# aquaskyline/SOAPdenovo-Trans

Hardware: AMD Instinct MI355X
Metric: pregraph k-mers hashed/sec (higher is better)
Workload: dtype u64

## Files before the change

soapdenovo-trans_amd/csrc/sdt_pipeline.hip:

```cpp
#include "sdt_ctx.hpp"
#include "sdt_tile.cuh"
#include "sdt_superkmer_kernels.cuh"
#include "sdt_count_plan.h"
#include "sdt_pipeline.hpp"

void sk_free(sdt_ctx *c)
{
	sdt_ctx::SkState &k = c->sk;
	void *dev[] = {k.p1.recs, k.p1.meta, k.p1.next, k.p2.recs, k.p2.meta, k.p2.next, k.cursors, k.blk, k.cnt1, k.off1, k.fill1, k.list1,
	               k.cnt2, k.off2, k.fill2, k.list2, k.kmers2, k.kpre2, k.items, k.citems, k.next_item};
	for (void *p : dev)
		if (p) (void)hipFree(p);
	void *host[] = {k.h_off1, k.h_off2, k.h_kpre2, k.h_items, k.h_citems};
	for (void *p : host)
		if (p) (void)hipHostFree(p);
	const uint64_t in_total = k.l2_in_total;
	const bool exchanged = k.exchanged;
	const uint32_t stream_flushes = k.stream_flushes;
	k = sdt_ctx::SkState();
	k.l2_in_total = in_total;
	k.exchanged = exchanged;
	k.stream_flushes = stream_flushes;
}

SkGeo sk_geo(int K, uint64_t max_read_len)
{
	SkGeo g;
	g.mtw = (int)(((uint64_t)SK_TILE_READS * max_read_len + 16 + 15) / 16) + TAIL_PAD + 1;
	g.tile_words = (int)((tile_smem_bytes(g.mtw) / sizeof(uint32_t) + 1) & ~(size_t)1);
	g.hv_words = (int)((SK_TILE_READS * max_read_len + 16 + 1) & ~(uint64_t)1);
	const uint64_t nk_max = (uint64_t)SK_TILE_READS * (max_read_len - K + 1);
	g.bits_words = (int)(nk_max / 64 + 2);
	g.hv2_words = K - sk_minimizer_len(K) + 1 > 49 ? g.hv_words : 0;
	g.smem = (size_t)g.tile_words * 4 + (size_t)SK_NB1 * 8 + (size_t)(g.hv_words + g.hv2_words) * 4 + (size_t)g.bits_words * 8 + (size_t)(g.bits_words + 2) * 4;
	return g;
}

template <int NW, bool TRACK> static size_t sk_count_smem()
{
	using G = SkCntGeo<NW, TRACK>;
	constexpr int SLOTS = G::SLOTS, BW = SkFmt<NW>::BW, TR = G::TILE;
	return (size_t)(NW + (TRACK ? 1 : 0)) * SLOTS * 8 + (size_t)TR * 8 + (size_t)SLOTS * 20 + (size_t)TR * 4 + G::REGION +
	       (size_t)(LDS_LEAD + TR * BW * 2 + TAIL_PAD) * 4;
}

bool sk_applicable(const sdt_ctx *c, uint64_t max_read_len)
{
	if (c->flags & SDT_FLAG_CONTIG_INDEX)
		return false;
	if (max_read_len < (uint64_t)c->K + 1 || max_read_len > (uint64_t)SK_MAX_READ_LEN)
		return false;
	return sk_geo(c->K, max_read_len).smem <= 160 * 1024;
}

int sk_reset_pool1(sdt_ctx *c)
{
	sdt_ctx::SkState &k = c->sk;
	HIPCHK(hipMemsetAsync(k.p1.next, 0, 4, c->stream));
	HIPCHK(hipMemsetAsync(k.cnt1, 0, SK_NB1 * 4, c->stream));
	hipLaunchKernelGGL(k_sk_init_cursors, dim3(256), dim3(256), 0, c->stream, k.cursors, k.wgs * (uint32_t)SK_NB1, (uint32_t)SK_CAP1, k.blk, k.wgs);
	HIPCHK(hipGetLastError());
	k.pending_kmers = 0;
	return SDT_OK;
}

int sk_alloc(sdt_ctx *c, uint64_t want_kmers, uint64_t per_read)
{
	sdt_ctx::SkState &k = c->sk;
	if (want_kmers > SK_BATCH_MAX_KMERS)
		want_kmers = SK_BATCH_MAX_KMERS;
	if (k.ready && (k.cap_kmers >= want_kmers || k.cap_is_max || k.pending_kmers))
		return SDT_OK;
	if (k.ready) {
		HIPCHK(hipStreamSynchronize(c->stream));
		sk_free(c);
	}
	const bool compact = sk_compact(c);
	const int rw = sk_rec_words(c->nw), rw2 = sk_rec2_stride(c->nw, compact);
	const int w = c->K - sk_minimizer_len(c->K) + 1;
	const bool strips = c->nw == 4 || per_read > (uint64_t)SK_SEQ_MAX_KMERS;
	const int cap_c = strips ? sk_pow2_floor(sk_max_run(c->K, c->nw, compact)) : sk_max_run(c->K, c->nw, compact);
	const double rate = 2.0 / (double)(w + 1) + 1.0 / (double)sk_max_run(c->K, c->nw);
	const double more = compact ? (2.0 / (double)(w + 1) + 1.0 / (double)cap_c) / rate : 1.0;
	double run = 1.0 / rate * ((c->nw == 4 || per_read > (uint64_t)SK_SEQ_MAX_KMERS) ? 0.8 : 1.0);
	if (run > (double)per_read) run = (double)per_read;
	uint64_t div = (uint64_t)run;
	if (div < 2) div = 2;
	div = (uint64_t)clamp_int(sdt_knob_int(sdt_tuning_env("SDT_SK_POOL_DIV"), (int)div), 1, 1 << 20);
	const int mem_pct = sdt_knob_int(sdt_tuning_env("SDT_SK_POOL_MEM_PCT"), 70);
	size_t free_b = 0, total_b = 0;
	HIPCHK(sdti::mem_info(&free_b, &total_b));
	uint64_t cap = want_kmers < (1ULL << 24) ? (1ULL << 24) : want_kmers;
	k.cap_is_max = cap >= SK_BATCH_MAX_KMERS;
	const uint32_t wgs = (uint32_t)c->cu_count * 6;
	for (;; cap /= 2) {
		const uint64_t recs = (uint64_t)((double)(cap / div) * more);
		const uint64_t chunks1 = sdt_knob_int(sdt_test_env("SDT_SK_POOL_CHUNKS1"), 0) > 0 ? (uint64_t)sdt_knob_int(sdt_test_env("SDT_SK_POOL_CHUNKS1"), 0) : recs / SK_CAP1 + (uint64_t)wgs * SK_NB1 + 1024;
		const uint64_t items = chunks1 / SK_ITEM_CHUNKS + SK_NB1 + 1;
		const uint64_t chunks2 = chunks1 * (SK_CAP1 / SK_CAP2) + items * (SK_NB2 + SK_BLK2) + 1024;
		const uint64_t bytes = chunks1 * SK_CAP1 * rw * 8 + chunks2 * SK_CAP2 * rw2 * 8 + (chunks1 + chunks2) * 8;
		const uint64_t all = c->comm.nranks > 1 ? bytes + chunks1 * SK_CAP1 * rw * 8 * 9 / 2 : bytes;
		if (chunks2 >= (1ULL << SK_LIST2_FILL_SHIFT) - 1 || all > free_b / 100 * (uint64_t)mem_pct) {
			k.cap_is_max = true;
			if (cap <= (1ULL << 24))
				return fail(SDT_ENOMEM, "super-k-mer pools: %llu MiB needed for the smallest batch, %zu MiB free",
				            (unsigned long long)(bytes >> 20), free_b >> 20);
			continue;
		}
		k.p1.chunks = (uint32_t)chunks1;
		k.p2.chunks = (uint32_t)chunks2;
		k.items_cap = (uint32_t)items;
		break;
	}
	k.wgs = wgs;
	const double t_alloc0 = comm_now();
	HIPCHK(hipMalloc((void **)&k.p1.recs, (size_t)k.p1.chunks * SK_CAP1 * rw * 8));
	HIPCHK(hipMalloc((void **)&k.p1.meta, (size_t)k.p1.chunks * 4));
	HIPCHK(hipMalloc((void **)&k.p1.next, 64));
	HIPCHK(hipMalloc((void **)&k.p2.recs, (size_t)k.p2.chunks * SK_CAP2 * rw2 * 8));
	HIPCHK(hipMalloc((void **)&k.p2.meta, (size_t)k.p2.chunks * 4));
	HIPCHK(hipMalloc((void **)&k.p2.next, 64));
	HIPCHK(hipMalloc((void **)&k.cursors, (size_t)wgs * SK_NB1 * 8));
	HIPCHK(hipMalloc((void **)&k.blk, (size_t)wgs * 8));
	HIPCHK(hipMalloc((void **)&k.cnt1, SK_NB1 * 4));
	HIPCHK(hipMalloc((void **)&k.off1, (SK_NB1 + 1) * 4));
	HIPCHK(hipMalloc((void **)&k.fill1, SK_NB1 * 4));
	HIPCHK(hipMalloc((void **)&k.list1, (size_t)k.p1.chunks * 4));
	HIPCHK(hipMalloc((void **)&k.cnt2, SK_NBF * 4));
	HIPCHK(hipMalloc((void **)&k.off2, (SK_NBF + 1) * 4));
	HIPCHK(hipMalloc((void **)&k.fill2, SK_NBF * 4));
	HIPCHK(hipMalloc((void **)&k.list2, (size_t)k.p2.chunks * 4));
	HIPCHK(hipMalloc((void **)&k.kmers2, SK_NBF * 8));
	HIPCHK(hipMalloc((void **)&k.kpre2, (SK_NBF + 1) * 8));
	HIPCHK(hipMalloc((void **)&k.items, (size_t)k.items_cap * sizeof(SkItem)));
	HIPCHK(hipHostMalloc((void **)&k.h_off1, (SK_NB1 + 1) * 4, hipHostMallocDefault));
	HIPCHK(hipHostMalloc((void **)&k.h_off2, (SK_NBF + 1) * 4, hipHostMallocDefault));
	HIPCHK(hipHostMalloc((void **)&k.h_kpre2, (SK_NBF + 1) * 8, hipHostMallocDefault));
	HIPCHK(hipHostMalloc((void **)&k.h_items, (size_t)k.items_cap * sizeof(SkItem), hipHostMallocDefault));
	k.citems_cap = (uint32_t)SK_NBF + k.p2.chunks / SK_COUNT_ITEM_CHUNKS + 1;
	HIPCHK(hipMalloc((void **)&k.citems, (size_t)k.citems_cap * sizeof(uint4)));
	HIPCHK(hipHostMalloc((void **)&k.h_citems, (size_t)k.citems_cap * sizeof(uint4), hipHostMallocDefault));
	HIPCHK(hipMalloc((void **)&k.next_item, SK_MAX_COUNT_LAUNCHES * sizeof(uint32_t)));
	k.cap_kmers = cap;
	k.ready = true;
	if (sdt_env("SDT_TIMING"))
		fprintf(stderr, "[libsdt_gpu] super-k-mer pools for %llu k-mers per batch: %.1f GiB in %.0f ms\n", (unsigned long long)cap,
		        ((double)k.p1.chunks * SK_CAP1 * rw + (double)k.p2.chunks * SK_CAP2 * rw2) * 8 / (1 << 30), (comm_now() - t_alloc0) * 1e3);
	return sk_reset_pool1(c);
}

template <int NW, bool TRACK, bool COMPACT> static int sk_launch_count_t(sdt_ctx *c, uint32_t i0, uint32_t i1, uint32_t launch)
{
	sdt_ctx::SkState &k = c->sk;
	const size_t smem = sk_count_smem<NW, TRACK>();
	const unsigned per_cu = (unsigned)((160 * 1024) / (smem + 256));
	unsigned grid = (unsigned)c->cu_count * (per_cu < 1 ? 1 : (per_cu > 2 ? 2 : per_cu));
	if (grid > i1 - i0) grid = i1 - i0;
	HIPCHK(hipFuncSetAttribute((const void *)k_sk_count<NW, TRACK, COMPACT>, hipFuncAttributeMaxDynamicSharedMemorySize, (int)smem));
	hipLaunchKernelGGL((k_sk_count<NW, TRACK, COMPACT>), dim3(grid), dim3(SkCntGeo<NW, TRACK>::TPB), smem, c->stream, k.p2, k.list2, (const uint4 *)k.citems, i0, i1,
	                   k.next_item + launch, c->K, flat_of<NW>(c), c->d_stats);
	HIPCHK(hipGetLastError());
	return SDT_OK;
}

template <int NW> static int sk_launch_count(sdt_ctx *c, uint32_t i0, uint32_t i1, uint32_t launch)
{
	if (c->d_first)
		return sk_launch_count_t<NW, true, false>(c, i0, i1, launch);
	if constexpr (NW == 1)
		if (sk_compact(c))
			return sk_launch_count_t<1, false, true>(c, i0, i1, launch);
	return sk_launch_count_t<NW, false, false>(c, i0, i1, launch);
}


int sk_list1(sdt_ctx *c)
{
	sdt_ctx::SkState &k = c->sk;
	const int g = c->cu_count * 8;
	hipLaunchKernelGGL(k_sk_seal, dim3(256), dim3(256), 0, c->stream, k.cursors, k.wgs * (uint32_t)SK_NB1, k.blk, k.wgs, k.p1, (uint32_t)SK_CAP1);
	hipLaunchKernelGGL(k_sk_scan, dim3(1), dim3(1024), 0, c->stream, k.cnt1, k.off1, k.fill1, (int)SK_NB1, (const unsigned long long *)nullptr, (unsigned long long *)nullptr);
	hipLaunchKernelGGL(k_sk_chunk_place_few, dim3(g), dim3(256), 0, c->stream, k.p1, k.off1, k.fill1, k.list1, (int)SK_NB1);
	SK_CHK(hipGetLastError());
	SK_CHK(hipMemcpyAsync(k.h_off1, k.off1, (SK_NB1 + 1) * 4, hipMemcpyDeviceToHost, c->stream));
	{ const int rcw = c->comm.sync_watched(c->stream, "the chunk lists of a round"); if (rcw != SDT_OK) return rcw; }
	k.st_chunks1 = k.h_off1[SK_NB1];
	return SDT_OK;
}

int sk_split(sdt_ctx *c, const SkPool &src, const uint32_t *list, uint32_t nitems, hipEvent_t after_l2)
{
	sdt_ctx::SkState &k = c->sk;
	const int g = c->cu_count * 8;
	SK_CHK(hipMemsetAsync(k.p2.next, 0, 4, c->stream));
	SK_CHK(hipMemsetAsync(k.kmers2, 0, SK_NBF * 8, c->stream));
	SK_CHK(hipMemsetAsync(k.cnt2, 0, SK_NBF * 4, c->stream));
	if (nitems) {
		SK_CHK(hipMemcpyAsync(k.items, k.h_items, (size_t)nitems * sizeof(SkItem), hipMemcpyHostToDevice, c->stream));
#define SK_L2_LAUNCH(NW, COMPACT)                                                                                                   \
		do {                                                                                                                        \
			const size_t sm = SkL2Stage<NW, COMPACT>::SMEM;                                                                         \
			SK_CHK(hipFuncSetAttribute((const void *)k_sk_scatter_records_staged<NW, COMPACT>, hipFuncAttributeMaxDynamicSharedMemorySize, (int)sm)); \
			hipLaunchKernelGGL((k_sk_scatter_records_staged<NW, COMPACT>), dim3(nitems), dim3(SK_L2S_TPB), sm, c->stream, src, list, k.items, k.p2, k.cnt2, k.kmers2, c->d_stats); \
		} while (0)
		if (c->nw == 1 && sk_compact(c)) SK_L2_LAUNCH(1, true);
		else if (c->nw == 1) SK_L2_LAUNCH(1, false);
		else if (c->nw == 2) SK_L2_LAUNCH(2, false);
		else SK_L2_LAUNCH(4, false);
#undef SK_L2_LAUNCH
		SK_CHK(hipGetLastError());
	}
	if (after_l2)
		SK_CHK(hipEventRecord(after_l2, c->stream));
	hipLaunchKernelGGL(k_sk_scan, dim3(1), dim3(1024), 0, c->stream, k.cnt2, k.off2, k.fill2, (int)SK_NBF, (const unsigned long long *)k.kmers2, k.kpre2);
	hipLaunchKernelGGL(k_sk_chunk_place, dim3(g), dim3(256), 0, c->stream, k.p2, k.off2, k.fill2, k.list2);
	SK_CHK(hipGetLastError());
	SK_CHK(hipMemcpyAsync(k.h_kpre2, k.kpre2, (SK_NBF + 1) * 8, hipMemcpyDeviceToHost, c->stream));
	SK_CHK(hipMemcpyAsync(k.h_off2, k.off2, (SK_NBF + 1) * 4, hipMemcpyDeviceToHost, c->stream));
	return SDT_OK;
}

int sk_count_all(sdt_ctx *c)
{
	sdt_ctx::SkState &k = c->sk;
	SK_CHK(hipStreamSynchronize(c->stream));
	k.st_chunks2 = k.h_off2[SK_NBF];
	k.st_flushes++;
	k.stream_flushes++;
	k.l2_in_total += k.h_kpre2[SK_NBF];
	int rc = SDT_OK;
	uint32_t nci = 0;
	SK_CHK(hipMemsetAsync(k.next_item, 0, SK_MAX_COUNT_LAUNCHES * sizeof(uint32_t), c->stream));
	std::vector<uint32_t> first_item(SK_MAX_COUNT_LAUNCHES + 2);
	std::vector<uint64_t> launch_kmers(SK_MAX_COUNT_LAUNCHES + 2);
	uint32_t nlaunches = 0;
	
	if (!sk_plan_count_items(k.h_off2, (const uint64_t *)k.h_kpre2, (uint32_t)SK_NBF, c->kmers_known == 0 ? (1ULL << 26) : SK_COUNT_KMERS, SK_COUNT_KMERS,
	                         SK_MAX_COUNT_LAUNCHES, SK_COUNT_PACK_CHUNKS, SK_COUNT_ITEM_CHUNKS, (uint32_t *)k.h_citems, k.citems_cap,
	                         first_item.data(), launch_kmers.data(), (uint32_t)first_item.size(), &nci, &nlaunches))
		return fail(SDT_ESTATE, "count stage: work item table overflow");
	first_item.resize(nlaunches + 1);
	launch_kmers.resize(nlaunches);
	std::vector<uint32_t> sort_tmp;
	auto guess_of = [&](uint64_t kmers) -> uint64_t {
		uint64_t bound = kmers;
		if (c->kmers_known) {
			const double rate = (double)c->distinct_known / (double)c->kmers_known;
			const uint64_t guess = (uint64_t)((double)kmers * (2.0 * rate < 1.0 ? 2.0 * rate : 1.0)) + (1ULL << 22);
			if (guess < bound) bound = guess;
		}
		return bound;
	};
	const size_t nl = first_item.size() - 1;
	for (size_t l = 0; l < nl && rc == SDT_OK;) {
		const uint32_t i0 = first_item[l];
		if (i0 == first_item[l + 1]) {
			l++;
			continue;
		}
		if (c->kmers_known == 0 && l > 0) {
			rc = sync_stats(c);
			if (rc != SDT_OK) break;
		}
		uint64_t bound = guess_of(launch_kmers[l]), hard = launch_kmers[l];
		rc = ensure_room(c, bound);
		if (rc == SDT_OK && (double)(c->distinct_known + c->hard_since_sync + launch_kmers[l]) > 0.95 * (double)c->slots) {
			rc = sync_stats(c);
			if (rc == SDT_OK && (double)(c->distinct_known + launch_kmers[l]) > 0.95 * (double)c->slots)
				rc = grow_table(c, c->distinct_known + launch_kmers[l]);
		}
		size_t m = l;
		while (rc == SDT_OK && c->kmers_known && m + 1 < nl) {
			const uint64_t b2 = guess_of(launch_kmers[m + 1]);
			if ((double)(c->distinct_known + c->kmers_since_sync + bound + b2) > (double)c->slots * MAX_LOAD)
				break;
			if ((double)(c->distinct_known + c->hard_since_sync + hard + launch_kmers[m + 1]) > 0.95 * (double)c->slots)
				break;
			bound += b2;
			hard += launch_kmers[m + 1];
			m++;
		}
		const uint32_t i1 = first_item[m + 1];
		if (m > l)
			sk_plan_largest_first((uint32_t *)k.h_citems, i0, i1, sort_tmp);
		if (rc == SDT_OK)
			SK_CHK(hipMemcpyAsync(k.citems + i0, k.h_citems + i0, (size_t)(i1 - i0) * sizeof(uint4), hipMemcpyHostToDevice, c->stream));
		if (rc == SDT_OK)
			rc = c->nw == 1 ? sk_launch_count<1>(c, i0, i1, (uint32_t)l) : c->nw == 2 ? sk_launch_count<2>(c, i0, i1, (uint32_t)l) : sk_launch_count<4>(c, i0, i1, (uint32_t)l);
		if (rc == SDT_OK) {
			c->kmers_since_sync += bound;
			c->hard_since_sync += hard;
		}
		l = m + 1;
	}
	return rc;
}

int sk_add_items(sdt_ctx::SkState &k, uint32_t &nitems, uint32_t b, uint32_t lo, uint32_t hi)
{
	for (uint32_t c0 = lo; c0 < hi; c0 += SK_ITEM_CHUNKS) {
		if (nitems >= k.items_cap)
			return fail(SDT_EHIP, "super-k-mer pipeline: item table overflow");
		k.h_items[nitems++] = SkItem{b, c0, c0 + SK_ITEM_CHUNKS < hi ? c0 + SK_ITEM_CHUNKS : hi, 0};
	}
	return SDT_OK;
}

int sk_flush_sharded(sdt_ctx *c);

int sk_flush(sdt_ctx *c)
{
	sdt_ctx::SkState &k = c->sk;
	if (!k.ready || k.pending_kmers == 0 || k.flushing)
		return SDT_OK;
	if (c->comm.nranks > 1)
		return fail(SDT_ESTATE, "sharded context: the pipeline is drained by the collective calls (sdt_gpu_count_reads_sharded)");
	k.flushing = true;
	EventPair *ev = next_event(c), *ev2 = next_event(c);
	if (!ev || !ev2) { k.flushing = false; return fail(SDT_EHIP, "hipEventCreate failed"); }
	ev = ev2 - 1;
	ev->kmers = ev2->kmers = 0;
	ev->stage = SDT_STAGE_SK_SPLIT;
	ev2->stage = SDT_STAGE_SK_COUNT;
	int rc = hipEventRecord(ev->a, c->stream) == hipSuccess ? SDT_OK : fail(SDT_EHIP, "hipEventRecord failed");
	if (rc == SDT_OK) rc = sk_list1(c);
	uint32_t nitems = 0;
	for (uint32_t b = 0; b < (uint32_t)SK_NB1 && rc == SDT_OK; b++)
		rc = sk_add_items(k, nitems, b, k.h_off1[b], k.h_off1[b + 1]);
	if (rc == SDT_OK) rc = sk_split(c, k.p1, k.list1, nitems, nullptr);
	if (rc == SDT_OK) rc = sk_reset_pool1(c);
	if (rc == SDT_OK && (hipEventRecord(ev->b, c->stream) != hipSuccess || hipEventRecord(ev2->a, c->stream) != hipSuccess))
		rc = fail(SDT_EHIP, "hipEventRecord failed");
	if (rc == SDT_OK) {
		k.pending_kmers = 0;
		rc = sk_count_all(c);
	}
	if (hipEventRecord(ev2->b, c->stream) != hipSuccess && rc == SDT_OK)
		rc = fail(SDT_EHIP, "hipEventRecord failed");
	k.flushing = false;
	return rc;
}

template <int NW> static Table<NW> sk_tbl(const sdt_ctx *c, bool allow_direct)
{
	Table<NW> t = flat_of<NW>(c);
	if (!allow_direct)
		t.ent = nullptr;
	return t;
}

int sk_scatter_launch(sdt_ctx *c, const uint32_t *d_words, const uint64_t *d_offs, uint64_t nr, uint64_t max_read_len, uint64_t ob,
                             bool allow_direct)
{
	sdt_ctx::SkState &k = c->sk;
	const uint64_t per_read = max_read_len - c->K + 1;
	const SkGeo geo = sk_geo(c->K, max_read_len);
	const int m = sk_minimizer_len(c->K), ncap = sk_max_run(c->K, c->nw, sk_compact(c));
	const uint64_t ntiles = (nr + SK_TILE_READS - 1) / SK_TILE_READS;
	const unsigned grid = (unsigned)(ntiles < k.wgs ? ntiles : k.wgs);
	EventPair *ev = next_event(c);
	if (!ev)
		return fail(SDT_EHIP, "hipEventCreate failed");
	ev->kmers = nr * per_read;
	ev->stage = SDT_STAGE_SK_SCATTER;
	HIPCHK(hipEventRecord(ev->a, c->stream));
#define SK_SCATTER(NW)                                                                                                             \
	do {                                                                                                                       \
		HIPCHK(hipFuncSetAttribute((const void *)k_sk_scatter_reads<NW>, hipFuncAttributeMaxDynamicSharedMemorySize, (int)geo.smem)); \
		hipLaunchKernelGGL(k_sk_scatter_reads<NW>, dim3(grid), dim3(TPB), geo.smem, c->stream, d_words, d_offs, nr, c->K, m, sk_pow2_floor(ncap), \
		                   geo.mtw, geo.tile_words, geo.hv_words, geo.hv2_words, geo.bits_words, k.p1, k.cursors, k.blk, k.cnt1, sk_tbl<NW>(c, allow_direct), c->d_stats, ob, c->ord_stride); \
	} while (0)
	const int w = c->K - m + 1;
	static const bool no_seq = sdt_tuning_env("SDT_SK_STRIPS") != NULL;
	const bool seq1 = c->nw == 1 && (w & 1) && w >= 9 && w <= 21 && per_read <= (uint64_t)SK_SEQ_MAX_KMERS;
	const bool seq2 = c->nw == 2 && (w & 1) && w >= 23 && w <= 53 && per_read <= (uint64_t)SK_SEQ_MAX_KMERS;
	if ((seq1 || seq2) && !no_seq) {
		SkSeqLaunch a;
		a.words = d_words; a.offs = d_offs; a.nreads = nr; a.K = c->K; a.m = m; a.ncap = ncap;
		a.mtw = (int)(((uint64_t)SK_SEQ_TILE * max_read_len + 16 + 15) / 16) + TAIL_PAD + 1;
		a.pool = k.p1; a.cursors = k.cursors; a.blk = k.blk; a.cnt = k.cnt1; a.stats = c->d_stats;
		a.ord_base = ob; a.ord_stride = c->ord_stride; a.max_wgs = k.wgs; a.cu_count = c->cu_count; a.stream = c->stream;
		HIPCHK(seq1 ? sk_seq_launch_nw1(w, a, sk_tbl<1>(c, allow_direct)) : (w <= 33 ? sk_seq_launch_nw2_lo(w, a, sk_tbl<2>(c, allow_direct))
		            : (w <= 43 ? sk_seq_launch_nw2_mid(w, a, sk_tbl<2>(c, allow_direct)) : sk_seq_launch_nw2_hi(w, a, sk_tbl<2>(c, allow_direct)))));
	} else if (c->nw == 1) SK_SCATTER(1);
	else if (c->nw == 2) SK_SCATTER(2);
	else SK_SCATTER(4);
#undef SK_SCATTER
	HIPCHK(hipGetLastError());
	HIPCHK(hipEventRecord(ev->b, c->stream));
	k.pending_kmers += nr * per_read;
	return SDT_OK;
}

uint64_t sk_batch_limit(const sdt_ctx *c)
{
	const sdt_ctx::SkState &k = c->sk;
	if (c->expect_kmers && c->expect_kmers / 16 >= (1ULL << 27) && k.stream_flushes < 4) {
		const uint64_t lim = (c->expect_kmers / 16) << k.stream_flushes;
		if (lim < k.cap_kmers)
			return lim;
	}
	return k.cap_kmers;
}

int sk_scatter(sdt_ctx *c, const uint32_t *d_words, const uint64_t *d_offs, uint64_t nreads, uint64_t max_read_len)
{
	sdt_ctx::SkState &k = c->sk;
	const uint64_t per_read = max_read_len - c->K + 1;
	int rc = SDT_OK;
	if (k.ready && k.pending_kmers && !k.cap_is_max && k.cap_kmers < k.pending_kmers + nreads * per_read && k.cap_kmers < (1ULL << 31))
		rc = sk_flush(c);
	if (rc == SDT_OK) {
		uint64_t want = k.pending_kmers + nreads * per_read;
		if (!(c->flags & SDT_FLAG_PARTITION) && want < (1ULL << 31))
			want = 1ULL << 31;
		if (c->expect_kmers > want) {
			const uint64_t lim = 1ULL << clamp_int(sdt_knob_int(sdt_tuning_env("SDT_SK_HINT_BATCH_LOG2"), 32), 24, 34);
			const uint64_t hinted = c->expect_kmers < lim ? c->expect_kmers : lim;
			if (hinted > want) want = hinted;
		}
		rc = sk_alloc(c, want, per_read);
	}
	if (rc != SDT_OK)
		return rc;
	for (uint64_t r0 = 0; r0 < nreads;) {
		if (k.pending_kmers + per_read * SK_TILE_READS > sk_batch_limit(c)) {
			rc = sk_flush(c);
			if (rc == SDT_OK && !k.cap_is_max && k.cap_kmers < (1ULL << 31))
				rc = sk_alloc(c, k.cap_kmers * 2, per_read);
			if (rc != SDT_OK)
				return rc;
		}
		uint64_t nr = (sk_batch_limit(c) - k.pending_kmers) / per_read / SK_TILE_READS * SK_TILE_READS;
		if (nr > nreads - r0) nr = nreads - r0;
		rc = sk_scatter_launch(c, d_words, d_offs + r0, nr, max_read_len, c->ord_base + r0 * c->ord_stride);
		if (rc != SDT_OK)
			return rc;
		r0 += nr;
	}
	return SDT_OK;
}

extern "C" {
int sdt_sk_plan_count_items(const uint32_t *off2, const uint64_t *kpre2, uint32_t nbuckets, uint64_t first_limit, uint64_t limit,
                            uint32_t max_launches, uint32_t *items, uint32_t items_cap, uint32_t *first_item, uint64_t *launch_kmers,
                            uint32_t launches_cap, uint32_t *nitems, uint32_t *nlaunches)
{
	if (!off2 || !kpre2 || !items || !first_item || !launch_kmers || !nitems || !nlaunches)
		return fail(SDT_EINVAL, "NULL argument");
	if (max_launches < 1 || limit == 0 || first_limit == 0)
		return fail(SDT_EINVAL, "bad argument (at least one launch, limits of at least one k-mer)");
	if (!sk_plan_count_items(off2, kpre2, nbuckets, first_limit, limit, max_launches, SK_COUNT_PACK_CHUNKS, SK_COUNT_ITEM_CHUNKS, items, items_cap,
	                         first_item, launch_kmers, launches_cap, nitems, nlaunches))
		return fail(SDT_ENOMEM, "output arrays too small");
	return SDT_OK;
}

int sdt_kmer_bucket(const uint64_t *key_words_msw_first, int K)
{
	if (!key_words_msw_first || K < 13 || K > 127)
		return -1;
	const int nw = K <= 31 ? 1 : (K <= 63 ? 2 : 4), m = sk_minimizer_len(K);
	uint32_t best = 0xFFFFFFFFu;
	for (int p = 0; p + m <= K; p++) {
		uint32_t fw = 0;
		for (int i = 0; i < m; i++) {
			const int bit = 2 * (K - 1 - (p + i));
			const uint64_t w = key_words_msw_first[nw - 1 - bit / 64];
			fw = (fw << 2) | (uint32_t)((w >> (bit % 64)) & 3u);
		}
		const uint32_t hv = sk_mmer_hash(sk_canon_mmer(fw, m));
		if (hv < best) best = hv;
	}
	return (int)sk_l1_bucket(sk_bucket_hash(best));
}

int sdt_kmer_final_bucket(const uint64_t *key_words_msw_first, int K)
{
	if (!key_words_msw_first || K < 13 || K > 127)
		return -1;
	if (K <= 31) { Key<1> k{{key_words_msw_first[0]}}; return (int)key_final_bucket<1>(k, K); }
	if (K <= 63) { Key<2> k{{key_words_msw_first[0], key_words_msw_first[1]}}; return (int)key_final_bucket<2>(k, K); }
	Key<4> k{{key_words_msw_first[0], key_words_msw_first[1], key_words_msw_first[2], key_words_msw_first[3]}};
	return (int)key_final_bucket<4>(k, K);
}
#ifdef SDT_SK_L2_LOG
extern "C" int sdt_gpu_debug_l2_log(sdt_ctx *c, void *d_buf, uint64_t cap)
{
	unsigned long long *p = (unsigned long long *)d_buf, cp = cap;
	HIPCHK(hipSetDevice(c->device));
	HIPCHK(hipMemcpyToSymbol(HIP_SYMBOL(g_l2_log), &p, sizeof p));
	HIPCHK(hipMemcpyToSymbol(HIP_SYMBOL(g_l2_log_cap), &cp, sizeof cp));
	return SDT_OK;
}
#endif
}
```

soapdenovo-trans_amd/csrc/sdt_pipeline.hpp:

```cpp
#pragma once
#include "sdt_ctx.hpp"

static const uint64_t SK_BATCH_MAX_KMERS = 1ULL << clamp_int(sdt_knob_int(sdt_size_env("SDT_SK_BATCH_LOG2"), 35), 24, 36);
static const uint32_t SK_ITEM_CHUNKS = (uint32_t)clamp_int(sdt_knob_int(sdt_size_env("SDT_SK_ITEM_CHUNKS"), 4096), 16, 4096);
static const uint64_t SK_COUNT_KMERS = 1ULL << clamp_int(sdt_knob_int(sdt_size_env("SDT_SK_COUNT_KMERS_LOG2"), 29), 20, 36);
static const uint32_t SK_COUNT_PACK_CHUNKS = 64;
static const uint32_t SK_COUNT_ITEM_CHUNKS = (uint32_t)clamp_int(sdt_knob_int(sdt_size_env("SDT_SK_COUNT_ITEM_CHUNKS"), 2048), 64, 1 << 24);
static const uint32_t SK_MAX_COUNT_LAUNCHES = 4096;


#define SK_CHK(expr)                                                                                   \
	do {                                                                                               \
		hipError_t e4_ = (expr);                                                                       \
		if (e4_ != hipSuccess)                                                                         \
			return fail(e4_ == hipErrorOutOfMemory ? SDT_ENOMEM : SDT_EHIP, "%s failed: %s (%s:%d)", #expr, hipGetErrorString(e4_), __FILE__, __LINE__); \
	} while (0)

static inline bool sk_compact(const sdt_ctx *c) { return sdt::sk_compact2(c->nw, (c->flags & SDT_FLAG_TRACK_FIRST) != 0); }

struct SkGeo { int mtw, tile_words, hv_words, hv2_words, bits_words; size_t smem; };
SkGeo sk_geo(int K, uint64_t max_read_len);
bool sk_applicable(const sdt_ctx *c, uint64_t max_read_len);
int sk_reset_pool1(sdt_ctx *c);
int sk_alloc(sdt_ctx *c, uint64_t want_kmers, uint64_t per_read);
int sk_list1(sdt_ctx *c);
int sk_split(sdt_ctx *c, const SkPool &src, const uint32_t *list, uint32_t nitems, hipEvent_t after_l2);
int sk_count_all(sdt_ctx *c);
int sk_add_items(sdt_ctx::SkState &k, uint32_t &nitems, uint32_t b, uint32_t lo, uint32_t hi);
int sk_scatter_launch(sdt_ctx *c, const uint32_t *d_words, const uint64_t *d_offs, uint64_t nr, uint64_t max_read_len, uint64_t ob,
                      bool allow_direct = true);
uint64_t sk_batch_limit(const sdt_ctx *c);
int sk_scatter(sdt_ctx *c, const uint32_t *d_words, const uint64_t *d_offs, uint64_t nreads, uint64_t max_read_len);
```

soapdenovo-trans_amd/csrc/sdt_scatter_seq_a.hip:

```cpp
#include "sdt_sk_scatter_seq.cuh"

hipError_t sk_seq_launch_nw1(int w, const SkSeqLaunch &a, const Table<1> &tbl)
{
	switch (w) {
	case 9: return sk_seq_launch_one<1, 9>(a, tbl);
	case 11: return sk_seq_launch_one<1, 11>(a, tbl);
	case 13: return sk_seq_launch_one<1, 13>(a, tbl);
	case 15: return sk_seq_launch_one<1, 15>(a, tbl);
	case 17: return sk_seq_launch_one<1, 17>(a, tbl);
	case 19: return sk_seq_launch_one<1, 19>(a, tbl);
	case 21: return sk_seq_launch_one<1, 21>(a, tbl);
	default: return hipErrorInvalidValue;
	}
}
```

soapdenovo-trans_amd/csrc/sdt_sharded.hip:

```cpp
#include "sdt_ctx.hpp"
#include "sdt_tile.cuh"
#include "sdt_superkmer_kernels.cuh"
#include "sdt_pipeline.hpp"

void shard_free(sdt_ctx *c)
{
	sdt_ctx::Shard &h = c->sh;
	for (int i = 0; i < 2; i++) {
		if (h.send[i]) (void)hipFree(h.send[i]);
		if (h.recv[i]) (void)hipFree(h.recv[i]);
		if (h.send_meta[i]) (void)hipFree(h.send_meta[i]);
		if (h.recv_meta[i]) (void)hipFree(h.recv_meta[i]);
		if (h.ev_gather[i]) (void)hipEventDestroy(h.ev_gather[i]);
		if (h.ev_xdone[i]) (void)hipEventDestroy(h.ev_xdone[i]);
		if (h.ev_l2[i]) (void)hipEventDestroy(h.ev_l2[i]);
	}
	if (h.iota) (void)hipFree(h.iota);
	h = sdt_ctx::Shard();
}

int shard_alloc(sdt_ctx *c)
{
	sdt_ctx::Shard &h = c->sh;
	sdt_ctx::SkState &k = c->sk;
	if (h.send[0] && h.send_chunks >= k.p1.chunks)
		return SDT_OK;
	HIPCHK(hipStreamSynchronize(c->stream));
	shard_free(c);
	const size_t cw = (size_t)SK_CAP1 * sk_rec_words(c->nw) * 8;
	h.send_chunks = k.p1.chunks;
	h.recv_chunks = k.p1.chunks + k.p1.chunks / 4;
	if (sdt_test_env("SDT_SHARD_RECV_CHUNKS"))
		h.recv_chunks = (uint32_t)strtoul(sdt_test_env("SDT_SHARD_RECV_CHUNKS"), nullptr, 10);
	for (int i = 0; i < 2; i++) {
		HIPCHK(hipMalloc((void **)&h.send[i], (size_t)h.send_chunks * cw));
		HIPCHK(hipMalloc((void **)&h.recv[i], (size_t)h.recv_chunks * cw));
		HIPCHK(hipMalloc((void **)&h.send_meta[i], (size_t)h.send_chunks * 4));
		HIPCHK(hipMalloc((void **)&h.recv_meta[i], (size_t)h.recv_chunks * 4));
		HIPCHK(hipEventCreateWithFlags(&h.ev_gather[i], hipEventDisableTiming));
		HIPCHK(hipEventCreateWithFlags(&h.ev_xdone[i], hipEventDisableTiming));
		HIPCHK(hipEventCreateWithFlags(&h.ev_l2[i], hipEventDisableTiming));
	}
	HIPCHK(hipMalloc((void **)&h.iota, (size_t)h.recv_chunks * 4));
	hipLaunchKernelGGL(k_sk_iota, dim3(1024), dim3(256), 0, c->stream, h.iota, h.recv_chunks);
	HIPCHK(hipGetLastError());
	return SDT_OK;
}

int shard_finish_pending(sdt_ctx *c)
{
	sdt_ctx::Shard &h = c->sh;
	sdt_ctx::SkState &k = c->sk;
	if (!h.pending)
		return SDT_OK;
	h.pending = false;
	const int slot = h.pending_slot;
	EventPair *ev = next_event(c), *ev2 = next_event(c);
	if (!ev || !ev2) return fail(SDT_EHIP, "hipEventCreate failed");
	ev = ev2 - 1;
	ev->kmers = ev2->kmers = 0;
	ev->stage = SDT_STAGE_SK_SPLIT;
	ev2->stage = SDT_STAGE_SK_COUNT;
	HIPCHK(hipStreamWaitEvent(c->stream, h.ev_xdone[slot], 0));
	HIPCHK(hipEventRecord(ev->a, c->stream));
	if (h.items.size() > k.items_cap)
		return fail(SDT_EHIP, "super-k-mer pipeline: item table overflow");
	memcpy(k.h_items, h.items.data(), h.items.size() * sizeof(SkItem));
	SkPool src = {h.recv[slot], h.recv_meta[slot], nullptr, h.recv_chunks};
	int rc = sk_split(c, src, h.iota, (uint32_t)h.items.size(), h.ev_l2[slot]);
	if (rc != SDT_OK) return rc;
	h.l2_recorded[slot] = true;
	HIPCHK(hipEventRecord(ev->b, c->stream));
	HIPCHK(hipEventRecord(ev2->a, c->stream));
	rc = sk_count_all(c);
	HIPCHK(hipEventRecord(ev2->b, c->stream));
	return rc;
}

int sk_flush_sharded(sdt_ctx *c)
{
	sdt_ctx::Shard &h = c->sh;
	sdt_ctx::SkState &k = c->sk;
	Comm &cm = c->comm;
	const int n = cm.nranks, me = cm.rank;
	k.exchanged = true;
	int rc = sk_list1(c);
	if (rc != SDT_OK) return rc;
	std::vector<uint32_t> mat((size_t)n * (SK_NB1 + 1));
	rc = cm.allgather_host(k.h_off1, mat.data(), (SK_NB1 + 1) * sizeof(uint32_t));
	if (rc != SDT_OK) return rc;
	auto M = [&](int r, uint32_t b) { return shard_mat(mat.data(), r, b); };
	const uint32_t *blo = h.ranges;
	const uint32_t S = shard_subrounds(mat.data(), n, blo, h.recv_chunks);
	const size_t cw = (size_t)SK_CAP1 * sk_rec_words(c->nw) * 8;
	for (uint32_t t = 0; t < S; t++) {
		const int slot = (int)(h.round & 1);
		ShardRound sr;
		shard_round(mat.data(), n, me, blo, t, S, sr);
		auto piece = [&](int s2, int d, uint32_t &lo, uint32_t &hi) { shard_piece(mat.data(), blo, s2, d, t, S, lo, hi); };
		SkGatherPlan plan;
		memset(&plan, 0, sizeof plan);
		plan.n = n;
		plan.self = me;
		std::vector<void *> sp(n), rp(n), smp(n), rmp(n);
		std::vector<size_t> sb(n, 0), rb(n, 0), smb(n, 0), rmb(n, 0), oboff((size_t)n * n, 0), obmoff((size_t)n * n, 0);
		const uint32_t send_at = sr.send_total, recv_at = sr.recv_total;
		std::vector<SkItem> cur;
		for (int p = 0; p < n; p++) {
			plan.begin[p] = sr.send_begin[p];
			plan.pre[p + 1] = plan.pre[p] + sr.send_count[p];
			plan.dst0[p] = sr.send_at[p];
			if (p != me) {
				sp[p] = (uint8_t *)h.send[slot] + (size_t)sr.send_at[p] * cw;
				smp[p] = h.send_meta[slot] + sr.send_at[p];
				sb[p] = (size_t)sr.send_count[p] * cw;
				smb[p] = (size_t)sr.send_count[p] * 4;
			}
		}
		for (int s2 = 0; s2 < n; s2++) {
			uint32_t lo, hi;
			piece(s2, me, lo, hi);
			const uint32_t at = sr.recv_at[s2];
			rp[s2] = (uint8_t *)h.recv[slot] + (size_t)at * cw;
			rmp[s2] = h.recv_meta[slot] + at;
			rb[s2] = (size_t)(hi - lo) * cw;
			rmb[s2] = (size_t)(hi - lo) * 4;
			for (uint32_t b = blo[me]; b < blo[me + 1] && rc == SDT_OK; b++) {
				const uint32_t x0 = M(s2, b) > lo ? M(s2, b) : lo, x1 = M(s2, b + 1) < hi ? M(s2, b + 1) : hi;
				for (uint32_t c0 = at + (x0 - lo); x1 > x0 && c0 < at + (x1 - lo); c0 += SK_ITEM_CHUNKS) {
					const uint32_t c1 = c0 + SK_ITEM_CHUNKS < at + (x1 - lo) ? c0 + SK_ITEM_CHUNKS : at + (x1 - lo);
					cur.push_back(SkItem{b, c0, c1, 0});
				}
			}
		}
		if (send_at > h.send_chunks || recv_at > h.recv_chunks)
			return fail(SDT_EFULL, "exchange buffers too small: %u / %u chunks to send, %u / %u to receive", send_at, h.send_chunks, recv_at, h.recv_chunks);
		if (cm.kind == 2)
			for (int s2 = 0; s2 < n; s2++) {
				size_t at = 0, mat_at = 0;
				for (int d = 0; d < n; d++) {
					if (d == s2) continue;
					uint32_t lo, hi;
					piece(s2, d, lo, hi);
					oboff[(size_t)s2 * n + d] = at;
					at += (size_t)(hi - lo) * cw;
				}
				for (int d = 0; d < n; d++) {
					if (d == s2) continue;
					uint32_t lo, hi;
					piece(s2, d, lo, hi);
					obmoff[(size_t)s2 * n + d] = at + mat_at;
					mat_at += (size_t)(hi - lo) * 4;
				}
			}
		if (h.x_recorded[slot])
			HIPCHK(hipStreamWaitEvent(c->stream, h.ev_xdone[slot], 0));
		if (plan.pre[n]) {
			const unsigned g = (unsigned)c->cu_count * 8;
			if (c->nw == 1) hipLaunchKernelGGL(k_sk_gather<SkFmt<1>::REC_WORDS>, dim3(g), dim3(256), 0, c->stream, k.p1, k.list1, plan, h.send[slot], h.send_meta[slot], h.recv[slot], h.recv_meta[slot]);
			else if (c->nw == 2) hipLaunchKernelGGL(k_sk_gather<SkFmt<2>::REC_WORDS>, dim3(g), dim3(256), 0, c->stream, k.p1, k.list1, plan, h.send[slot], h.send_meta[slot], h.recv[slot], h.recv_meta[slot]);
			else hipLaunchKernelGGL(k_sk_gather<SkFmt<4>::REC_WORDS>, dim3(g), dim3(256), 0, c->stream, k.p1, k.list1, plan, h.send[slot], h.send_meta[slot], h.recv[slot], h.recv_meta[slot]);
			HIPCHK(hipGetLastError());
		}
		HIPCHK(hipEventRecord(h.ev_gather[slot], c->stream));
		if (t + 1 == S) {
			rc = sk_reset_pool1(c);
			if (rc != SDT_OK) return rc;
		}
		HIPCHK(hipStreamWaitEvent(cm.xstream, h.ev_gather[slot], 0));
		if (h.l2_recorded[slot])
			HIPCHK(hipStreamWaitEvent(cm.xstream, h.ev_l2[slot], 0));
		{
			void *const *const sps[2] = {sp.data(), smp.data()}, *const *const rps[2] = {rp.data(), rmp.data()};
			const size_t *const sbs[2] = {sb.data(), smb.data()}, *const rbs[2] = {rb.data(), rmb.data()}, *const obs[2] = {oboff.data(), obmoff.data()};
			rc = cm.exchange(2, sps, sbs, rps, rbs, obs);
		}
		if (rc != SDT_OK) return rc;
		HIPCHK(hipEventRecord(h.ev_xdone[slot], cm.xstream));
		h.x_recorded[slot] = true;
		rc = shard_finish_pending(c);
		if (rc != SDT_OK) return rc;
		h.items.swap(cur);
		h.pending = true;
		h.pending_slot = slot;
		h.round++;
	}
	return SDT_OK;
}

extern "C" {
int sdt_gpu_comm_id(sdt_comm_id *id)
{
	if (!id)
		return fail(SDT_EINVAL, "NULL argument");
	int rc = rccl_load();
	if (rc != SDT_OK)
		return rc;
	static_assert(sizeof(sdt_comm_id) == sizeof(NcclId), "ncclUniqueId is 128 bytes");
	NCCLCHK(g_rccl.GetUniqueId((NcclId *)id));
	return SDT_OK;
}

int sdt_gpu_comm_init(sdt_ctx *c, const sdt_comm_id *id, int rank, int nranks)
{
	if (!c || !id || nranks < 1 || nranks > 64 || rank < 0 || rank >= nranks)
		return fail(SDT_EINVAL, "bad argument (1..64 ranks)");
	if (c->comm.kind)
		return fail(SDT_ESTATE, "the context already has a communicator");
	HIPCHK(hipSetDevice(c->device));
	return c->comm.open_rccl((const NcclId *)id, rank, nranks);
}

int sdt_gpu_comm_init_shm(sdt_ctx *c, const char *name, int rank, int nranks)
{
	if (!c || !name || nranks < 1 || nranks > 64 || rank < 0 || rank >= nranks)
		return fail(SDT_EINVAL, "bad argument (1..64 ranks)");
	if (c->comm.kind)
		return fail(SDT_ESTATE, "the context already has a communicator");
	HIPCHK(hipSetDevice(c->device));
	return c->comm.open_shm(name, rank, nranks, true);
}

int sdt_comm_selftest_shm(const char *name, int rank, int nranks, int rounds)
{
	Comm cm;
	int rc = cm.open_shm(name, rank, nranks, false);
	if (rc != SDT_OK)
		return rc;
	for (int it = 0; it < rounds && rc == SDT_OK; it++) {
		std::vector<uint32_t> mine(257), all((size_t)257 * nranks);
		for (int i = 0; i < 257; i++) mine[i] = (uint32_t)(rank * 1000003 + it * 7919 + i);
		rc = cm.allgather_host(mine.data(), all.data(), 257 * sizeof(uint32_t));
		for (int r = 0; r < nranks && rc == SDT_OK; r++)
			for (int i = 0; i < 257; i++)
				if (all[(size_t)r * 257 + i] != (uint32_t)(r * 1000003 + it * 7919 + i))
					rc = fail(SDT_EHIP, "all-gather: rank %d got a wrong word from rank %d in round %d", rank, r, it);
		int64_t v[3] = {rank + 1, it, (int64_t)1 << 40};
		if (rc == SDT_OK) rc = cm.allreduce_sum_host(v, 3);
		if (rc == SDT_OK && (v[0] != (int64_t)nranks * (nranks + 1) / 2 || v[1] != (int64_t)it * nranks || v[2] != ((int64_t)nranks << 40)))
			rc = fail(SDT_EHIP, "all-reduce: rank %d got wrong sums in round %d", rank, it);
	}
	cm.close_all();
	return rc;
}

int sdt_gpu_allreduce_i64(sdt_ctx *c, int64_t *vals, int n)
{
	if (!c || !vals || n < 0 || (size_t)n * sizeof(int64_t) > SHM_CTRL_BYTES)
		return fail(SDT_EINVAL, "bad argument");
	HIPCHK(hipSetDevice(c->device));
	return c->comm.allreduce_sum_host(vals, n);
}

int sdt_gpu_comm_stats(sdt_ctx *c, uint64_t *bytes_sent, uint64_t *bytes_recv, double *exchange_ms, uint64_t *exchanges)
{
	if (!c)
		return fail(SDT_EINVAL, "ctx is NULL");
	HIPCHK(hipSetDevice(c->device));
	if (c->comm.xstream)
		HIPCHK(hipStreamSynchronize(c->comm.xstream));
	c->comm.harvest_time();
	if (bytes_sent) *bytes_sent = c->comm.bytes_sent;
	if (bytes_recv) *bytes_recv = c->comm.bytes_recv;
	if (exchange_ms) *exchange_ms = c->comm.exchange_ms;
	if (exchanges) *exchanges = c->comm.exchanges;
	return SDT_OK;
}

int sdt_gpu_shard_ranges(const sdt_ctx *c, uint32_t *first_bucket)
{
	if (!c || !first_bucket)
		return fail(SDT_EINVAL, "NULL argument");
	if (!c->sh.have_ranges)
		return fail(SDT_ESTATE, "no sharded call yet: the bucket ranges are cut on the first one");
	for (int r = 0; r <= c->comm.nranks; r++)
		first_bucket[r] = c->sh.ranges[r];
	return SDT_OK;
}

int sdt_shard_cut_ranges(const uint32_t *mat, int nranks, uint32_t *ranges)
{
	if (!mat || !ranges || nranks < 1 || nranks > SHARD_MAX_RANKS)
		return fail(SDT_EINVAL, "bad argument (1..64 ranks)");
	shard_cut_ranges(mat, nranks, ranges);
	return SDT_OK;
}

int sdt_shard_plan(const uint32_t *mat, int nranks, int me, const uint32_t *ranges, uint32_t recv_chunks, uint32_t t,
                   uint32_t *subrounds, uint32_t *send_begin, uint32_t *send_count, uint32_t *send_at, uint32_t *recv_count,
                   uint32_t *recv_at)
{
	if (!mat || !ranges || !subrounds || !send_begin || !send_count || !send_at || !recv_count || !recv_at)
		return fail(SDT_EINVAL, "NULL argument");
	if (nranks < 1 || nranks > SHARD_MAX_RANKS || me < 0 || me >= nranks || recv_chunks == 0)
		return fail(SDT_EINVAL, "bad argument (1..64 ranks, a receive buffer of at least one chunk)");
	const uint32_t S = shard_subrounds(mat, nranks, ranges, recv_chunks);
	*subrounds = S;
	if (t >= S)
		return fail(SDT_EINVAL, "sub-round %u of %u", t, S);
	ShardRound r;
	shard_round(mat, nranks, me, ranges, t, S, r);
	for (int p = 0; p < nranks; p++) {
		send_begin[p] = r.send_begin[p]; send_count[p] = r.send_count[p]; send_at[p] = r.send_at[p];
		recv_count[p] = r.recv_count[p]; recv_at[p] = r.recv_at[p];
	}
	return SDT_OK;
}
int sdt_kmer_owner(const uint64_t *key_words_msw_first, int K, int nranks)
{
	const int b = sdt_kmer_bucket(key_words_msw_first, K);
	if (b < 0 || nranks < 1)
		return -1;
	return sk_owner_of_bucket((uint32_t)b, nranks);
}
int sdt_gpu_count_reads_sharded(sdt_ctx *c, const void *d_packed_words, uint64_t nwords, const void *d_offsets, uint64_t nreads,
                                uint64_t max_read_len)
{
	(void)nwords;
	if (!c || (nreads && (!d_packed_words || !d_offsets)))
		return fail(SDT_EINVAL, "NULL argument");
	if (c->comm.kind == 0 || c->comm.nranks == 1) {
		if (nreads == 0)
			return SDT_OK;
		return sdt_gpu_count_reads_device(c, d_packed_words, nwords, d_offsets, nreads, max_read_len);
	}
	HIPCHK(hipSetDevice(c->device));
	{ const int rcd = drain_pushes(c, true); if (rcd != SDT_OK) return rcd; }
	Comm &cm = c->comm;
	sdt_ctx::SkState &k = c->sk;
	std::vector<uint64_t> all((size_t)2 * cm.nranks);
	uint64_t mine[2] = {nreads, nreads ? max_read_len : 0};
	int rc = cm.allgather_host(mine, all.data(), sizeof mine);
	if (rc != SDT_OK) return rc;
	uint64_t maxlen = 0, maxreads = 0;
	for (int r = 0; r < cm.nranks; r++) {
		if (all[2 * r] > maxreads) maxreads = all[2 * r];
		if (all[2 * r + 1] > maxlen) maxlen = all[2 * r + 1];
	}
	if (maxreads == 0 || maxlen < (uint64_t)c->K + 1) {
		c->ord_base += nreads * c->ord_stride;
		return SDT_OK;
	}
	if (maxlen > (uint64_t)SK_MAX_READ_LEN || sk_geo(c->K, maxlen).smem > 160 * 1024)
		return fail(SDT_EINVAL, "reads of %llu bases do not fit the LDS tile of the sharded path", (unsigned long long)maxlen);
	if (c->ord_base + nreads * c->ord_stride >= SK_MAX_READ_ORDINAL)
		return fail(SDT_EINVAL, "read ordinals past 2^34 do not fit a super-k-mer record");
	const uint64_t per_read = maxlen - c->K + 1;
	uint64_t want = maxreads * per_read;
	if (want > (1ULL << 31)) want = 1ULL << 31;
	if (sdt_test_env("SDT_SHARD_ROUND_KMERS"))
		want = strtoull(sdt_test_env("SDT_SHARD_ROUND_KMERS"), nullptr, 10);
	if (!k.ready || k.cap_kmers < want) {
		if (k.ready && !k.cap_is_max) { HIPCHK(hipStreamSynchronize(c->stream)); sk_free(c); }
		rc = sk_alloc(c, want, per_read);
		if (rc != SDT_OK) return rc;
	}
	rc = shard_alloc(c);
	if (rc != SDT_OK) return rc;
	if (!c->sh.have_ranges) {
		const uint64_t sample = nreads < (1ULL << 18) ? nreads : (1ULL << 18);
		if (sample) {
			rc = sk_scatter_launch(c, (const uint32_t *)d_packed_words, (const uint64_t *)d_offsets, sample, maxlen, c->ord_base, false);
			if (rc != SDT_OK) return rc;
		}
		rc = sk_list1(c);
		if (rc != SDT_OK) return rc;
		std::vector<uint32_t> mat((size_t)cm.nranks * (SK_NB1 + 1));
		rc = cm.allgather_host(k.h_off1, mat.data(), (SK_NB1 + 1) * sizeof(uint32_t));
		if (rc != SDT_OK) return rc;
		shard_cut_ranges(mat.data(), cm.nranks, c->sh.ranges);
		c->sh.have_ranges = true;
		rc = sk_reset_pool1(c);
		if (rc != SDT_OK) return rc;
	}
	uint64_t capmine = k.cap_kmers;
	std::vector<uint64_t> caps(cm.nranks);
	rc = cm.allgather_host(&capmine, caps.data(), sizeof capmine);
	if (rc != SDT_OK) return rc;
	uint64_t cap = caps[0];
	for (int r = 1; r < cm.nranks; r++) if (caps[r] < cap) cap = caps[r];
	if (sdt_test_env("SDT_SHARD_ROUND_KMERS") && cap > want) cap = want;
	uint64_t per_round = cap / per_read / SK_TILE_READS * SK_TILE_READS;
	if (per_round < (uint64_t)SK_TILE_READS) per_round = SK_TILE_READS;
	const uint64_t rounds = (maxreads + per_round - 1) / per_round;
	for (uint64_t i = 0; i < rounds; i++) {
		const uint64_t r0 = i * per_round;
		const uint64_t nr = r0 < nreads ? (nreads - r0 < per_round ? nreads - r0 : per_round) : 0;
		if (nr) {
			rc = sk_scatter_launch(c, (const uint32_t *)d_packed_words, (const uint64_t *)d_offsets + r0, nr, maxlen, c->ord_base + r0 * c->ord_stride, false);
			if (rc != SDT_OK) return rc;
			c->sh.kmers_scattered += nr * per_read;
		}
		k.flushing = true;
		rc = sk_flush_sharded(c);
		k.flushing = false;
		if (rc != SDT_OK) return rc;
	}
	k.flushing = true;
	rc = shard_finish_pending(c);
	k.flushing = false;
	c->ord_base += nreads * c->ord_stride;
	return rc;
}

int sdt_gpu_push_reads_sharded(sdt_ctx *c, const uint32_t *packed_words, uint64_t nwords, const uint64_t *offsets, uint64_t nreads)
{
	if (!c || (nreads && (!packed_words || !offsets)))
		return fail(SDT_EINVAL, "NULL argument");
	HIPCHK(hipSetDevice(c->device));
	uint64_t maxlen = 0;
	for (uint64_t i = 0; i < nreads; i++) {
		if (offsets[i + 1] < offsets[i])
			return fail(SDT_EINVAL, "offsets not monotonic at read %llu", (unsigned long long)i);
		if (offsets[i + 1] - offsets[i] > maxlen) maxlen = offsets[i + 1] - offsets[i];
	}
	if (nreads && ((offsets[nreads] + 15) >> 4) + TAIL_PAD > nwords)
		return fail(SDT_EINVAL, "packed_words too short");
	{ const int rcd = drain_pushes(c, true); if (rcd != SDT_OK) return rcd; }
	uint32_t *dw = nullptr;
	uint64_t *dof = nullptr;
	if (nreads) {
		HIPCHK(hipStreamSynchronize(c->stream));
		if (c->cap_words[0] < nwords) {
			if (c->d_words[0]) HIPCHK(hipFree(c->d_words[0]));
			c->d_words[0] = nullptr; c->cap_words[0] = 0;
			HIPCHK(hipMalloc((void **)&c->d_words[0], nwords * sizeof(uint32_t)));
			c->cap_words[0] = nwords;
		}
		if (c->cap_offs[0] < nreads + 1) {
			if (c->d_offs[0]) HIPCHK(hipFree(c->d_offs[0]));
			c->d_offs[0] = nullptr; c->cap_offs[0] = 0;
			HIPCHK(hipMalloc((void **)&c->d_offs[0], (nreads + 1) * sizeof(uint64_t)));
			c->cap_offs[0] = nreads + 1;
		}
		dw = c->d_words[0]; dof = c->d_offs[0];
		HIPCHK(hipMemcpyAsync(dw, packed_words, nwords * sizeof(uint32_t), hipMemcpyHostToDevice, c->stream));
		HIPCHK(hipMemcpyAsync(dof, offsets, (nreads + 1) * sizeof(uint64_t), hipMemcpyHostToDevice, c->stream));
	}
	const int rc = sdt_gpu_count_reads_sharded(c, dw, nwords, dof, nreads, maxlen);
	if (rc == SDT_OK)
		HIPCHK(hipStreamSynchronize(c->stream));
	return rc;
}
}
```

soapdenovo-trans_amd/csrc/sdt_sk_scatter_seq.cuh:

```cuda
#pragma once
#include <hip/hip_runtime.h>
#include "sdt_kmer.cuh"
#include "sdt_table.cuh"
#include "sdt_superkmer.cuh"

using namespace sdt;

constexpr uint32_t SK_BLK = 128;
#ifndef SDT_SK_BLK2
#define SDT_SK_BLK2 1024
#endif
constexpr uint32_t SK_BLK2 = SDT_SK_BLK2;
constexpr uint32_t SK_DEAD = 0xFFFFFFFFu;

#ifdef SDT_SK_L2_LOG
extern __device__ unsigned long long *g_l2_log;
extern __device__ unsigned long long g_l2_log_cap;
__device__ inline void sk_log_alloc(uint32_t path, uint32_t end, uint32_t id)
{
	if (g_l2_log) {
		const unsigned long long at = atomicAdd(g_l2_log, 1ULL);
		if (at + 1 < g_l2_log_cap)
			g_l2_log[1 + at] = (1ULL << 63) | ((unsigned long long)path << 61) | ((unsigned long long)(threadIdx.x & 0x1FFF) << 48) |
			                   ((unsigned long long)(end & 0xFFFFFFu) << 24) | (unsigned long long)(id & 0xFFFFFFu);
	}
}
__device__ inline void sk_log_cursor(uint32_t kind, uint32_t lb, uint32_t chunk, uint32_t pos)
{
	if (g_l2_log) {
		const unsigned long long at = atomicAdd(g_l2_log, 1ULL);
		if (at + 1 < g_l2_log_cap)
			g_l2_log[1 + at] = (1ULL << 63) | (3ULL << 61) | ((unsigned long long)kind << 59) | ((unsigned long long)(blockIdx.x & 15u) << 55) |
			                   ((unsigned long long)(threadIdx.x & 1023u) << 45) | ((unsigned long long)(lb & 1023u) << 35) |
			                   ((unsigned long long)(pos > 31u ? 31u : pos) << 30) | (unsigned long long)(chunk & 0x3FFFFFFFu);
	}
}
#else
__device__ inline void sk_log_alloc(uint32_t, uint32_t, uint32_t) {}
__device__ inline void sk_log_cursor(uint32_t, uint32_t, uint32_t, uint32_t) {}
#endif

__device__ inline uint32_t sk_alloc_chunk(unsigned long long *s_blk, const SkPool &pool, uint32_t blk = SK_BLK)
{
	uint32_t got = 0;
	bool done = false;
	while (!done) {
		{
			const unsigned long long w = __hip_atomic_load(s_blk, __ATOMIC_RELAXED, __HIP_MEMORY_SCOPE_WORKGROUP);
			if ((uint32_t)w > (uint32_t)(w >> 32)) {
				__builtin_amdgcn_s_sleep(1);
				continue;
			}
		}
		const unsigned long long v = atomicAdd(s_blk, 1ULL);
		const uint32_t id = (uint32_t)v, end = (uint32_t)(v >> 32);
		if (id < end) {
			got = id;
			done = true;
			sk_log_alloc(0, end, id);
		} else if (id == end) {
			const uint32_t base = atomicAdd(pool.next, blk);
			atomicExch(s_blk, ((unsigned long long)(base + blk) << 32) | (unsigned long long)(base + 1u));
			got = base;
			done = true;
			sk_log_alloc(1, end, base);
		}
	}
	return got;
}

__device__ inline uint32_t sk_alloc_chunks(unsigned long long *s_blk, const SkPool &pool, uint32_t n, uint32_t blk)
{
	uint32_t got = SK_NOCHUNK;
	bool done = false;
	while (!done) {
		{
			const unsigned long long w = __hip_atomic_load(s_blk, __ATOMIC_RELAXED, __HIP_MEMORY_SCOPE_WORKGROUP);
			if ((uint32_t)w > (uint32_t)(w >> 32)) {
				__builtin_amdgcn_s_sleep(1);
				continue;
			}
		}
		const unsigned long long v = atomicAdd(s_blk, (unsigned long long)n);
		const uint32_t id = (uint32_t)v, end = (uint32_t)(v >> 32);
		if (id <= end && id + n <= end) {
			got = id;
			done = true;
		} else if (id <= end) {
			for (uint32_t x = id; x < end && x < pool.chunks; x++)
				pool.meta[x] = SK_DEAD;
			const uint32_t base = atomicAdd(pool.next, n + blk);
			atomicExch(s_blk, ((unsigned long long)(base + n + blk) << 32) | (unsigned long long)(base + n));
			got = base;
			done = true;
		}
	}
	return got;
}

__device__ inline void sk_retire_block(unsigned long long blk, const SkPool &pool)
{
	const uint32_t next = (uint32_t)blk, end = (uint32_t)(blk >> 32);
	for (uint32_t id = next; id < end && id < pool.chunks; id++)
		pool.meta[id] = SK_DEAD;
}

__device__ inline bool sk_reserve(unsigned long long *s_cur, unsigned long long *s_blk, uint32_t lb, uint32_t meta_bucket,
                                  uint32_t cap, const SkPool &pool, uint32_t *s_cnt, uint32_t &chunk, uint32_t &pos)
{
	bool done = false, ok = false;
	while (!done) {
		if ((uint32_t)__hip_atomic_load(&s_cur[lb], __ATOMIC_RELAXED, __HIP_MEMORY_SCOPE_WORKGROUP) > cap) {
			__builtin_amdgcn_s_sleep(1);
			continue;
		}
		const unsigned long long cur = atomicAdd(&s_cur[lb], 1ULL);
		pos = (uint32_t)cur;
		chunk = (uint32_t)(cur >> 32);
		if (pos < cap) {
			ok = chunk != SK_NOCHUNK;
			done = true;
			sk_log_cursor(0, lb, chunk, pos);
		} else if (pos == cap) {
			sk_log_cursor(1, lb, chunk, pos);
			uint32_t id = sk_alloc_chunk(s_blk, pool);
			if (id >= pool.chunks) {
				id = SK_NOCHUNK;
			} else {
				pool.meta[id] = meta_bucket | (cap << 24);
				atomicAdd(&s_cnt[lb], 1u);
			}
			atomicExch(&s_cur[lb], ((unsigned long long)id << 32) | 1ULL);
			chunk = id;
			pos = 0;
			ok = id != SK_NOCHUNK;
			done = true;
			sk_log_cursor(3, lb, id, 1);
		} else {
#if SDT_SK_L2_LOG >= 2
			sk_log_cursor(2, lb, chunk, pos);
#endif
		}
	}
	return ok;
}

template <int RW> __device__ inline void sk_store_record(uint64_t *dst, const uint64_t (&rec)[RW])
{
#pragma unroll
	for (int i = 0; i < RW; i++)
		dst[i] = rec[i];
}
template <int NW> __device__ inline void sk_store_record2(uint64_t *dst, const uint64_t (&rec)[SkFmt<NW>::REC_WORDS])
{
	if constexpr (SkFmt<NW>::REC2_STRIDE == 4 && SkFmt<NW>::REC_WORDS == 3) {
		ulonglong2 *d = reinterpret_cast<ulonglong2 *>(dst);
		d[0] = make_ulonglong2(rec[0], rec[1]);
		d[1] = make_ulonglong2(rec[2], 0ULL);
	} else {
		sk_store_record<SkFmt<NW>::REC_WORDS>(dst, rec);
	}
}
template <int RW> __device__ inline void sk_load_record(const uint64_t *src, uint64_t (&rec)[RW])
{
#pragma unroll
	for (int i = 0; i < RW; i++)
		rec[i] = src[i];
}


constexpr int SK_SEQ_TILE = 256;
constexpr int SK_SEQ_RUNCAP = 24;
constexpr int SK_SEQ_MAX_KMERS = 256;


template <int NW>
__device__ inline void sk_emit_run(const uint32_t *words, int rb_r, int len_r, int nk_r, int K, uint64_t read_ord, int j0, int n,
                                   uint32_t fb, unsigned long long *s_cur, unsigned long long *s_blk, const SkPool &pool,
                                   uint32_t *s_cnt, const Table<NW> &tbl, uint32_t &claimed, uint32_t &failed, uint32_t &done,
                                   uint32_t &emitted)
{
	constexpr int BW = SkFmt<NW>::BW, RW = SkFmt<NW>::REC_WORDS;
	const int hp = j0 > 0, hn = j0 + n < nk_r;
	const uint32_t l1 = fb >> SK_L2BITS, l2 = fb & (SK_NB2 - 1);
	uint32_t chunk, pos;
	if (sk_reserve(s_cur, s_blk, l1, l1, SK_CAP1, pool, s_cnt, chunk, pos)) {
		const int len = hp + n + K - 1 + hn, ps = rb_r + j0 - hp;
		uint64_t rec[RW];
		rec[0] = sk_header(read_ord, (uint32_t)j0, l2, n, hp, hn);
#pragma unroll
		for (int k = 0; k < BW; k++) {
			uint64_t wv = 0;
			if (32 * k < len) {
				wv = sk_stream_word(words, ps + 32 * k);
				const int keep = len - 32 * k;
				if (keep < 32)
					wv &= ~0ULL << (64 - 2 * keep);
			}
			rec[1 + k] = wv;
		}
		sk_store_record<RW>(pool.recs + ((size_t)chunk * SK_CAP1 + pos) * RW, rec);
		emitted += (uint32_t)n;
	} else if (!tbl.ent) {
		failed += (uint32_t)n;
	} else {
		for (int jj = j0; jj < j0 + n; jj++) {
			uint32_t prev, next;
			const Key<NW> key = chop_record<NW>(words, rb_r, len_r, jj, K, prev, next);
			const uint64_t ord = tbl.first ? (read_ord << 16) | (uint64_t)jj : ORD_NONE;
			if (!table_put<NW>(tbl, key, prev, next, claimed, ord))
				failed++;
			done++;
		}
	}
}

template <int NW, int W>
__global__ __launch_bounds__(SK_SEQ_TILE, NW == 1 ? 4 : 2) void k_sk_scatter_reads_seq(const uint32_t *__restrict__ packed, const uint64_t *__restrict__ offs,
                                                                      uint64_t nreads, int K, int m, int ncap, int max_tile_words, SkPool pool,
                                                                      unsigned long long *__restrict__ g_cursors, unsigned long long *__restrict__ g_blk,
                                                                      uint32_t *__restrict__ g_cnt, Table<NW> tbl, Stats *stats,
                                                                      uint64_t ord_base, uint64_t ord_stride)
{
	constexpr int TR = SK_SEQ_TILE;
	extern __shared__ uint32_t smem[];
	unsigned long long *s_cur = (unsigned long long *)smem;
	uint32_t *s_rb = (uint32_t *)(s_cur + SK_NB1);
	uint32_t *s_runs = s_rb + TR + 2;
	uint32_t *s_words = s_runs + TR * SK_SEQ_RUNCAP;
	__shared__ unsigned long long s_blk;
	__shared__ uint32_t s_cnt[SK_NB1];
	const int tid = threadIdx.x;
	for (int i = tid; i < SK_NB1; i += TR) {
		s_cur[i] = g_cursors[(size_t)blockIdx.x * SK_NB1 + i];
		s_cnt[i] = 0;
	}
	if (tid == 0)
		s_blk = g_blk[blockIdx.x];
	const uint64_t ntiles = (nreads + TR - 1) / TR;
	const uint32_t mmask = (1u << (2 * m)) - 1u;
	const int topsh = 2 * (m - 1);
	uint32_t claimed = 0, failed = 0, done = 0, emitted = 0;
#ifdef SDT_SK_TICKS
	unsigned long long cyc[4] = {0, 0, 0, 0}, t0 = wall_clock64(), t1;
#define SK_TICK(i) do { t1 = wall_clock64(); cyc[i] += t1 - t0; t0 = t1; } while (0)
#else
#define SK_TICK(i) do { } while (0)
#endif
	for (uint64_t tile = blockIdx.x; tile < ntiles; tile += gridDim.x) {
		const uint64_t r0 = tile * TR;
		const int nr = (int)((nreads - r0) < (uint64_t)TR ? (nreads - r0) : (uint64_t)TR);
		const uint64_t word0 = offs[r0] >> 4;
		int nwords = (int)(((offs[r0 + nr] + 15) >> 4) - word0) + TAIL_PAD;
		if (nwords > max_tile_words)
			nwords = max_tile_words;
		s_rb[tid] = (uint32_t)(offs[r0 + (tid < nr ? tid : nr)] - (word0 << 4));
		if (tid == 0)
			s_rb[TR] = (uint32_t)(offs[r0 + nr] - (word0 << 4));
		if (tid < LDS_LEAD)
			s_words[tid] = 0;
		for (int i = tid; i < nwords; i += TR)
			s_words[LDS_LEAD + i] = packed[word0 + i];
		__syncthreads();
		SK_TICK(0);
		const uint32_t *words = s_words + LDS_LEAD;
		const int rb_r = (int)s_rb[tid];
		const int len_r = tid < nr ? (int)s_rb[tid + 1] - rb_r : 0;
		const int nk_r = len_r >= K + 1 ? len_r - K + 1 : 0;
		const uint64_t read_ord = ord_base + (r0 + (uint64_t)tid) * ord_stride;
		uint32_t *runs = s_runs + tid * SK_SEQ_RUNCAP;
		int nrun = 0;
		if (nk_r > 0) {
			const int nhv = len_r - m + 1;
			uint32_t fw = sk_stream_mmer(words, rb_r, m) >> 2;
			uint32_t rc = (sk_rev2bit32(fw ^ 0xAAAAAAAAu) >> (32 - 2 * (m - 1))) << 2;
			int pb = rb_r + m - 1;
			auto next_hv = [&]() -> uint32_t {
				const uint32_t b = (words[pb >> 4] >> (30 - 2 * (pb & 15))) & 3u;
				pb++;
				fw = ((fw << 2) | b) & mmask;
				rc = (rc >> 2) | ((b ^ 2u) << topsh);
				return sk_mmer_hash(fw < rc ? fw : rc);
			};
			int j0 = 0;
			uint32_t fb0 = 0, pfb = 0;
			auto window = [&](int j, uint32_t mn) {
				const uint32_t fb = sk_final_bucket(sk_bucket_hash(mn));
				if (j == 0) {
					fb0 = fb;
				} else if (j - j0 >= ncap || fb != pfb) {
					if (nrun < SK_SEQ_RUNCAP)
						runs[nrun] = (fb0 << 6) | (uint32_t)(j - j0 - 1);
					else
						sk_emit_run<NW>(words, rb_r, len_r, nk_r, K, read_ord, j0, j - j0, fb0, s_cur, &s_blk, pool, s_cnt, tbl, claimed, failed, done, emitted);
					nrun++;
					j0 = j;
					fb0 = fb;
				}
				pfb = fb;
			};
			uint32_t h[W], nh[W];
#pragma clang loop unroll(full)
			for (int i = 0; i < W; i++)
				h[i] = next_hv();
#pragma clang loop unroll(full)
			for (int i = W - 2; i >= 0; i--)
				h[i] = h[i] < h[i + 1] ? h[i] : h[i + 1];
			int p = W;
			for (int jb = 0; jb < nk_r; jb += W) {
				window(jb, h[0]);
				uint32_t pre = 0xFFFFFFFFu;
#pragma clang loop unroll(full)
				for (int i = 1; i < W; i++) {
					const uint32_t x = p < nhv ? next_hv() : 0xFFFFFFFFu;
					p++;
					nh[i - 1] = x;
					pre = x < pre ? x : pre;
					if (jb + i < nk_r)
						window(jb + i, h[i] < pre ? h[i] : pre);
				}
				nh[W - 1] = p < nhv ? next_hv() : 0xFFFFFFFFu;
				p++;
				h[W - 1] = nh[W - 1];
#pragma clang loop unroll(full)
				for (int i = W - 2; i >= 0; i--)
					h[i] = nh[i] < h[i + 1] ? nh[i] : h[i + 1];
			}
			if (nrun < SK_SEQ_RUNCAP)
				runs[nrun] = (fb0 << 6) | (uint32_t)(nk_r - j0 - 1);
			else
				sk_emit_run<NW>(words, rb_r, len_r, nk_r, K, read_ord, j0, nk_r - j0, fb0, s_cur, &s_blk, pool, s_cnt, tbl, claimed, failed, done, emitted);
			nrun++;
		}
		SK_TICK(1);
		const int nlist = nrun < SK_SEQ_RUNCAP ? nrun : SK_SEQ_RUNCAP;
		for (int k = 0, jr = 0; k < nlist; k++) {
			const uint32_t e = runs[k];
			const int nr = (int)(e & 63u) + 1;
			sk_emit_run<NW>(words, rb_r, len_r, nk_r, K, read_ord, jr, nr, e >> 6, s_cur, &s_blk, pool, s_cnt, tbl, claimed, failed, done, emitted);
			jr += nr;
		}
		__syncthreads();
		SK_TICK(3);
	}
#undef SK_TICK
	for (int i = tid; i < SK_NB1; i += TR) {
		g_cursors[(size_t)blockIdx.x * SK_NB1 + i] = s_cur[i];
		if (s_cnt[i])
			atomicAdd(&g_cnt[i], s_cnt[i]);
	}
	if (tid == 0) {
		g_blk[blockIdx.x] = s_blk;
#ifdef SDT_SK_TICKS
		for (int i = 0; i < 4; i++)
			atomicAdd(&stats->sk_cyc1[i], cyc[i]);
#endif
	}
	if (done) {
		atomicAdd(&stats->kmers, (unsigned long long)done);
		atomicAdd(&stats->sk_direct, (unsigned long long)done);
	}
	if (claimed) atomicAdd(&stats->distinct, (unsigned long long)claimed);
	if (failed) atomicAdd(&stats->probe_fail, (unsigned long long)failed);
#pragma unroll
	for (int d = 32; d > 0; d >>= 1)
		emitted += __shfl_down(emitted, d);
	if ((tid & 63) == 0 && emitted)
		atomicAdd(&stats->sk_emitted, (unsigned long long)emitted);
}


struct SkSeqLaunch {
	const uint32_t *words;
	const uint64_t *offs;
	uint64_t nreads;
	int K, m, ncap, mtw;
	SkPool pool;
	unsigned long long *cursors, *blk;
	uint32_t *cnt;
	Stats *stats;
	uint64_t ord_base, ord_stride;
	unsigned max_wgs;
	int cu_count;
	hipStream_t stream;
};

template <int NW, int W> inline hipError_t sk_seq_launch_one(const SkSeqLaunch &a, const Table<NW> &tbl)
{
	const size_t smem = (size_t)SK_NB1 * 8 + (size_t)(SK_SEQ_TILE + 2) * 4 + (size_t)SK_SEQ_TILE * SK_SEQ_RUNCAP * 4 + (size_t)(LDS_LEAD + a.mtw) * 4;
	hipError_t e = hipFuncSetAttribute((const void *)k_sk_scatter_reads_seq<NW, W>, hipFuncAttributeMaxDynamicSharedMemorySize, (int)smem);
	if (e != hipSuccess) return e;
	int per_cu = 0;
	e = hipOccupancyMaxActiveBlocksPerMultiprocessor(&per_cu, k_sk_scatter_reads_seq<NW, W>, SK_SEQ_TILE, smem);
	if (e != hipSuccess) return e;
	uint64_t res = (uint64_t)(per_cu > 0 ? per_cu : 1) * (uint64_t)a.cu_count;
	if (res > a.max_wgs) res = a.max_wgs;
	const uint64_t nt = (a.nreads + SK_SEQ_TILE - 1) / SK_SEQ_TILE;
	const unsigned grid = (unsigned)(nt < res ? nt : res);
	hipLaunchKernelGGL((k_sk_scatter_reads_seq<NW, W>), dim3(grid), dim3(SK_SEQ_TILE), smem, a.stream, a.words, a.offs, a.nreads, a.K, a.m, a.ncap,
	                   a.mtw, a.pool, a.cursors, a.blk, a.cnt, tbl, a.stats, a.ord_base, a.ord_stride);
	return hipGetLastError();
}

hipError_t sk_seq_launch_nw1(int w, const SkSeqLaunch &a, const Table<1> &tbl);
hipError_t sk_seq_launch_nw2_lo(int w, const SkSeqLaunch &a, const Table<2> &tbl);
hipError_t sk_seq_launch_nw2_mid(int w, const SkSeqLaunch &a, const Table<2> &tbl);
hipError_t sk_seq_launch_nw2_hi(int w, const SkSeqLaunch &a, const Table<2> &tbl);
```

soapdenovo-trans_amd/csrc/sdt_superkmer.cuh:

```cuda
#pragma once
#include "sdt_kmer.cuh"
#include "sdt_minimizer.cuh"
#include "sdt_table.cuh"
#include "sdt_sk_record2.h"

namespace sdt {

constexpr int SK_POSBITS = 22 - SK_L2BITS;
constexpr int SK_CAP1 = 32;
#ifndef SDT_SK_CAP2
#define SDT_SK_CAP2 16
#endif
constexpr int SK_CAP2 = SDT_SK_CAP2;
static_assert(SK_CAP2 == 16 || SK_CAP2 == 32, "a level-2 chunk holds 16 or 32 records");
constexpr uint32_t SK_NOCHUNK = 0xFFFFFFFFu;

template <int NW> struct SkFmt {
	static constexpr int BW = NW == 1 ? 2 : (NW == 2 ? 4 : 6);
	static constexpr int REC_WORDS = 1 + BW;
	static constexpr int CAP_BASES = 32 * BW;
#ifndef SDT_SK_REC2_PAD
#define SDT_SK_REC2_PAD 0
#endif
	static constexpr int REC2_STRIDE = (NW == 1 && SDT_SK_REC2_PAD) ? 4 : REC_WORDS;
};
constexpr uint64_t SK_MAX_READ_ORDINAL = 1ULL << 34;
constexpr int SK_MAX_READ_LEN = (1 << SK_POSBITS) - 1;

__host__ __device__ inline int sk_rec_words(int nw) { return nw == 1 ? 3 : (nw == 2 ? 5 : 7); }
__host__ __device__ inline int sk_rec2_stride(int nw, bool compact)
{
	return compact ? SK_REC2C_WORDS : (nw == 1 ? SkFmt<1>::REC2_STRIDE : (nw == 2 ? SkFmt<2>::REC2_STRIDE : SkFmt<4>::REC2_STRIDE));
}

__host__ __device__ inline uint32_t sk_stream_mmer(const uint32_t *words, int p, int m)
{
	const int s = 2 * p, wi = s >> 5, sh = s & 31;
	const uint64_t win = ((uint64_t)words[wi] << 32) | words[wi + 1];
	return (uint32_t)((win << sh) >> (64 - 2 * m));
}

__host__ __device__ inline uint64_t sk_stream_word(const uint32_t *words, int p)
{
	const int s = 2 * p, wi = s >> 5, sh = s & 31;
	const uint64_t hi = ((uint64_t)words[wi] << 32) | words[wi + 1];
	return sh ? ((hi << sh) | ((uint64_t)words[wi + 2] >> (32 - sh))) : hi;
}

__host__ __device__ inline uint64_t sk_header(uint64_t read_ord, uint32_t pos, uint32_t l2, int n, int has_prev, int has_next)
{
	return (read_ord << 30) | ((uint64_t)(pos & (uint32_t)SK_MAX_READ_LEN) << (8 + SK_L2BITS)) | ((uint64_t)(l2 & (uint32_t)(SK_NB2 - 1)) << 8) | ((uint64_t)(n - 1) << 2) |
	       ((uint64_t)has_prev << 1) | (uint64_t)has_next;
}
__host__ __device__ inline int sk_hdr_n(uint64_t h) { return (int)((h >> 2) & 63u) + 1; }
__host__ __device__ inline int sk_hdr_prev(uint64_t h) { return (int)((h >> 1) & 1u); }
__host__ __device__ inline int sk_hdr_next(uint64_t h) { return (int)(h & 1u); }
__host__ __device__ inline uint32_t sk_hdr_l2(uint64_t h) { return (uint32_t)((h >> 8) & (uint32_t)(SK_NB2 - 1)); }
__host__ __device__ inline uint32_t sk_hdr_pos(uint64_t h) { return (uint32_t)((h >> (8 + SK_L2BITS)) & (uint32_t)SK_MAX_READ_LEN); }
__host__ __device__ inline uint64_t sk_hdr_read(uint64_t h) { return h >> 30; }
static_assert(SK_L2BITS >= 10 && SK_L2BITS <= 12, "the record header holds a 10..12-bit level-2 bucket");
constexpr uint32_t SK_HDR_KIND_MASK = (1u << (8 + SK_L2BITS)) - 1u;

struct SkItem { uint32_t b1, c0, c1, pad; };
constexpr int SK_TILE_READS = 32;
struct SkPool {
	uint64_t *recs;
	uint32_t *meta;
	uint32_t *next;
	uint32_t chunks;
};

}
```

soapdenovo-trans_amd/csrc/sdt_superkmer_kernels.cuh:

```cuda
#pragma once

#ifndef SDT_SK_PREFETCH
#define SDT_SK_PREFETCH 1
#endif
#ifndef SDT_SK_CLAIM_BELOW
#define SDT_SK_CLAIM_BELOW 0
#endif
#ifndef SDT_SK_LOAD16
#define SDT_SK_LOAD16 1
#endif
#ifndef SDT_SK_CLAIM2_BELOW
#define SDT_SK_CLAIM2_BELOW 0
#endif
#ifndef SDT_SK_FLUSH_NUM
#define SDT_SK_FLUSH_NUM 4
#endif
#ifndef SDT_SK_NW2_TWO
#define SDT_SK_NW2_TWO 1
#endif
#ifndef SDT_SK_SEQ_FLUSH
#define SDT_SK_SEQ_FLUSH 1
#endif
#ifndef SDT_SK_CNT_TPB
#define SDT_SK_CNT_TPB 1024
#endif
#ifndef SDT_SK_SLOTS_TRACK
#define SDT_SK_SLOTS_TRACK 1536
#endif
#ifndef SDT_SK_SLOTS_NW2
#define SDT_SK_SLOTS_NW2 1280
#endif
#ifndef SDT_SK_SLOTS_NW1
#define SDT_SK_SLOTS_NW1 2048
#endif
template <int NW, bool TRACK> struct SkCntGeo {
	static constexpr int TPB = SDT_SK_CNT_TPB;
	static constexpr int WAVES_PER_SIMD = (NW == 1 || (NW == 2 && SDT_SK_NW2_TWO)) ? 2 * (TPB / 256) : TPB / 256;
	static constexpr int TILE = 512;
#ifdef SDT_SK_TEST_SLOTS
	static constexpr int SLOTS = SDT_SK_TEST_SLOTS;
#else
	static constexpr int SLOTS = NW == 1 ? (TRACK ? SDT_SK_SLOTS_TRACK : SDT_SK_SLOTS_NW1) : (NW == 2 ? SDT_SK_SLOTS_NW2 : 2048);
#endif
	static constexpr int FLUSH_AT = SLOTS * SDT_SK_FLUSH_NUM / 8;
	static constexpr int MAXFILL = SLOTS - 8;
	static constexpr int MAXN = NW == 1 ? 32 : 64;
	static constexpr int IDXN = TILE * MAXN / 16;
	static constexpr int REP = 2 * TILE;
	static constexpr size_t REGION = (((size_t)(TILE + 2) * 4 + (size_t)TILE * 2 + (size_t)IDXN * 2) + 7) & ~(size_t)7;
	static_assert(((LDS_LEAD + TAIL_PAD) & 1) == 0, "the LDS table behind the tile's words is 8-byte aligned");
	static_assert(REGION >= (size_t)REP * 4, "the dedupe table aliases prefix + map + index");
};
#ifndef SDT_SK_L2S_TPB
#define SDT_SK_L2S_TPB 1024
#endif
constexpr int SK_L2S_TPB = SDT_SK_L2S_TPB;
constexpr int SK_LIST2_FILL_SHIFT = SK_CAP2 == 16 ? 28 : 27;

#include "sdt_sk_scatter_seq.cuh"

template <int NW>
__global__ __launch_bounds__(TPB) void k_sk_scatter_reads(const uint32_t *__restrict__ packed, const uint64_t *__restrict__ offs,
                                                          uint64_t nreads, int K, int m, int ncap, int max_tile_words,
                                                          int tile_smem_words, int hv_words, int hv2_words, int bits_words, SkPool pool,
                                                          unsigned long long *__restrict__ g_cursors, unsigned long long *__restrict__ g_blk,
                                                          uint32_t *__restrict__ g_cnt, Table<NW> tbl, Stats *stats,
                                                          uint64_t ord_base, uint64_t ord_stride)
{
	constexpr int BW = SkFmt<NW>::BW, RW = SkFmt<NW>::REC_WORDS;
	extern __shared__ uint32_t smem[];
	unsigned long long *s_cur = (unsigned long long *)(smem + tile_smem_words);
	uint32_t *s_hv = (uint32_t *)(s_cur + SK_NB1);
	uint32_t *s_hv2 = s_hv + hv_words;
	unsigned long long *s_bits = (unsigned long long *)(s_hv2 + hv2_words);
	uint32_t *s_pc = (uint32_t *)(s_bits + bits_words);
	__shared__ unsigned long long s_blk;
	__shared__ uint32_t s_cnt[SK_NB1];
	const int tid = threadIdx.x;
	for (int i = tid; i < SK_NB1; i += TPB) {
		s_cur[i] = g_cursors[(size_t)blockIdx.x * SK_NB1 + i];
		s_cnt[i] = 0;
	}
	if (tid == 0)
		s_blk = g_blk[blockIdx.x];
	const int w = K - m + 1;
	const uint64_t ntiles = (nreads + SK_TILE_READS - 1) / SK_TILE_READS;
	uint32_t claimed = 0, failed = 0, done = 0, emitted = 0;
#ifdef SDT_SK_TICKS
	unsigned long long cyc[4] = {0, 0, 0, 0}, t0 = wall_clock64(), t1;
#define SK_TICK(i) do { t1 = wall_clock64(); cyc[i] += t1 - t0; t0 = t1; } while (0)
#else
#define SK_TICK(i) do { } while (0)
#endif
	for (uint64_t tile = blockIdx.x; tile < ntiles; tile += gridDim.x) {
		for (int i = tid; i < bits_words; i += TPB)
			s_bits[i] = 0;
		const TileView tv = stage_tile(smem, max_tile_words, packed, offs, tile * SK_TILE_READS, nreads, K, SK_TILE_READS);
		const int npos = (int)tv.rb[tv.nr];
		SK_TICK(0);
		const bool strips = w <= 49;
		const uint32_t *bhs = s_hv;
		const uint32_t nk = tv.nk, nkr = (nk + 63u) & ~63u;
		if (strips) {
			const int valid = 64 - w, lane = tid & 63;
			int P = 1;
			while (2 * P <= w)
				P *= 2;
			for (int r = tid >> 6; r < tv.nr; r += TPB / 64) {
				const int nk_r = (int)(tv.pre[r + 1] - tv.pre[r]);
				const int rb_r = (int)tv.rb[r], len_r = (int)tv.rb[r + 1] - rb_r;
				for (int j0 = 0; j0 < nk_r; j0 += valid) {
					const int j = j0 + lane - 1, p = rb_r + j;
					uint32_t x = (j >= 0 && j + m <= len_r) ? sk_mmer_hash(sk_canon_mmer(sk_stream_mmer(tv.words, p, m), m)) : 0xFFFFFFFFu;
					for (int d = 1; d < P; d <<= 1) {
						const uint32_t y = __shfl_down(x, d);
						x = y < x ? y : x;
					}
					const uint32_t y = __shfl_down(x, w - P);
					x = y < x ? y : x;
					const uint32_t bh = sk_bucket_hash(x), pbh = __shfl_up(bh, 1);
					const bool kv = lane >= 1 && lane <= valid && j < nk_r;
					if (kv)
						s_hv[p] = bh;
					const bool start = kv && (j == 0 || (j & (ncap - 1)) == 0 || sk_final_bucket(bh) != sk_final_bucket(pbh));
					const unsigned long long mask = __ballot(start) >> 1;
					if (lane == 0 && mask) {
						const uint32_t q0 = tv.pre[r] + (uint32_t)j0, sh = q0 & 63u;
						atomicOr(&s_bits[q0 >> 6], mask << sh);
						if (sh && (mask >> (64u - sh)))
							atomicOr(&s_bits[(q0 >> 6) + 1], mask >> (64u - sh));
					}
				}
			}
		} else {
			for (int p = tid; p < npos; p += TPB)
				s_hv[p] = p + m <= npos ? sk_mmer_hash(sk_canon_mmer(sk_stream_mmer(tv.words, p, m), m)) : 0xFFFFFFFFu;
			__syncthreads();
			int P = 1;
			while (2 * P <= w)
				P *= 2;
			uint32_t *src = s_hv, *dst = s_hv2;
			for (int d = 1; d < P; d <<= 1) {
				for (int p = tid; p < npos; p += TPB) {
					const uint32_t a = src[p], b = p + d < npos ? src[p + d] : 0xFFFFFFFFu;
					dst[p] = b < a ? b : a;
				}
				__syncthreads();
				uint32_t *t = src; src = dst; dst = t;
			}
			for (int p = tid; p < npos; p += TPB) {
				const uint32_t a = src[p], b = p + w - P < npos ? src[p + w - P] : 0xFFFFFFFFu;
				dst[p] = sk_bucket_hash(b < a ? b : a);
			}
			__syncthreads();
			bhs = dst;
			for (uint32_t q = tid; q < nkr; q += TPB) {
				bool start = false;
				if (q < nk) {
					const int r = tile_find_read(tv.pre, q);
					const int j = (int)(q - tv.pre[r]);
					const int p = (int)tv.rb[r] + j;
					if (j == 0 || (j & (ncap - 1)) == 0) {
						start = true;
					} else {
						start = sk_final_bucket(bhs[p]) != sk_final_bucket(bhs[p - 1]);
					}
				}
				const unsigned long long mask = __ballot(start);
				if ((tid & 63) == 0)
					s_bits[q >> 6] = mask;
			}
		}
		__syncthreads();
		SK_TICK(1);
		const int nw64 = (int)(nkr >> 6);
		if (tid < 64) {
			uint32_t run = 0;
			for (int base = 0; base < nw64; base += 64) {
				const int i = base + tid;
				const uint32_t c = i < nw64 ? (uint32_t)__popcll(s_bits[i]) : 0u;
				uint32_t x = c;
#pragma unroll
				for (int d = 1; d < 64; d <<= 1) {
					const uint32_t y = __shfl_up(x, d);
					if (tid >= d)
						x += y;
				}
				if (i < nw64)
					s_pc[i] = run + x - c;
				run += __shfl(x, 63);
			}
			if (tid == 0)
				s_pc[nw64] = run;
		}
		__syncthreads();
		const uint32_t ns = nw64 ? s_pc[nw64] : 0u;
		SK_TICK(2);
		for (uint32_t i = tid; i < ns; i += TPB) {
			int lo = 0, hi = nw64;
			while (hi - lo > 1) {
				const int mid = (lo + hi) >> 1;
				if (s_pc[mid] <= i) lo = mid; else hi = mid;
			}
			unsigned long long x = s_bits[lo];
			for (uint32_t k = i - s_pc[lo]; k; k--)
				x &= x - 1;
			const uint32_t q = (uint32_t)lo * 64u + (uint32_t)(__ffsll((long long)x) - 1);
			const unsigned long long rest = x & (x - 1);
			uint32_t qn;
			if (rest) {
				qn = (uint32_t)lo * 64u + (uint32_t)(__ffsll((long long)rest) - 1);
			} else {
				int wd = lo + 1;
				while (wd < nw64 && s_bits[wd] == 0)
					wd++;
				qn = wd < nw64 ? (uint32_t)wd * 64u + (uint32_t)(__ffsll((long long)s_bits[wd]) - 1) : nk;
			}
			const int n = (int)(qn - q);
			const int r = tile_find_read(tv.pre, q);
			const int j = (int)(q - tv.pre[r]);
			const int nk_r = (int)(tv.pre[r + 1] - tv.pre[r]);
			const int p0 = (int)tv.rb[r] + j;
			const int hp = j > 0, hn = j + n < nk_r;
			const uint32_t bh = bhs[p0];
			const uint64_t read_ord = ord_base + (tile * SK_TILE_READS + (uint64_t)r) * ord_stride;
			uint32_t chunk, pos;
			if (sk_reserve(s_cur, &s_blk, sk_l1_bucket(bh), sk_l1_bucket(bh), SK_CAP1, pool, s_cnt, chunk, pos)) {
				const int len = hp + n + K - 1 + hn, ps = p0 - hp;
				uint64_t rec[RW];
				rec[0] = sk_header(read_ord, (uint32_t)j, sk_l2_bucket(bh), n, hp, hn);
#pragma unroll
				for (int k = 0; k < BW; k++) {
					uint64_t wv = 0;
					if (32 * k < len) {
						wv = sk_stream_word(tv.words, ps + 32 * k);
						const int keep = len - 32 * k;
						if (keep < 32)
							wv &= ~0ULL << (64 - 2 * keep);
					}
					rec[1 + k] = wv;
				}
				sk_store_record<RW>(pool.recs + ((size_t)chunk * SK_CAP1 + pos) * RW, rec);
				emitted += (uint32_t)n;
			} else if (!tbl.ent) {
				failed += (uint32_t)n;
			} else {
				const int len_r = (int)(tv.rb[r + 1] - tv.rb[r]);
				for (int jj = j; jj < j + n; jj++) {
					uint32_t prev, next;
					const Key<NW> key = chop_record<NW>(tv.words, (int)tv.rb[r], len_r, jj, K, prev, next);
					const uint64_t ord = tbl.first ? (read_ord << 16) | (uint64_t)jj : ORD_NONE;
					if (!table_put<NW>(tbl, key, prev, next, claimed, ord))
						failed++;
					done++;
				}
			}
		}
		__syncthreads();
		SK_TICK(3);
	}
#undef SK_TICK
	for (int i = tid; i < SK_NB1; i += TPB) {
		g_cursors[(size_t)blockIdx.x * SK_NB1 + i] = s_cur[i];
		if (s_cnt[i])
			atomicAdd(&g_cnt[i], s_cnt[i]);
	}
	if (tid == 0) {
		g_blk[blockIdx.x] = s_blk;
#ifdef SDT_SK_TICKS
		for (int i = 0; i < 4; i++)
			atomicAdd(&stats->sk_cyc1[i], cyc[i]);
#endif
	}
	if (done) {
		atomicAdd(&stats->kmers, (unsigned long long)done);
		atomicAdd(&stats->sk_direct, (unsigned long long)done);
	}
	if (claimed) atomicAdd(&stats->distinct, (unsigned long long)claimed);
	if (failed) atomicAdd(&stats->probe_fail, (unsigned long long)failed);
#pragma unroll
	for (int d = 32; d > 0; d >>= 1)
		emitted += __shfl_down(emitted, d);
	if ((tid & 63) == 0 && emitted)
		atomicAdd(&stats->sk_emitted, (unsigned long long)emitted);
}

static __global__ __launch_bounds__(256) void k_sk_seal(const unsigned long long *__restrict__ cursors, uint32_t n, const unsigned long long *__restrict__ blk,
                                                 uint32_t nblk, SkPool pool, uint32_t cap)
{
	for (uint32_t i = blockIdx.x * 256u + threadIdx.x; i < n; i += gridDim.x * 256u) {
		const unsigned long long cur = cursors[i];
		const uint32_t chunk = (uint32_t)(cur >> 32), pos = (uint32_t)cur;
		if (chunk != SK_NOCHUNK)
			pool.meta[chunk] = (pool.meta[chunk] & 0xFFFFFFu) | ((pos < cap ? pos : cap) << 24);
	}
	for (uint32_t i = blockIdx.x * 256u + threadIdx.x; i < nblk; i += gridDim.x * 256u)
		sk_retire_block(blk[i], pool);
}

static __global__ __launch_bounds__(256) void k_sk_init_cursors(unsigned long long *cursors, uint32_t n, uint32_t cap, unsigned long long *blk, uint32_t nblk)
{
	for (uint32_t i = blockIdx.x * 256u + threadIdx.x; i < n; i += gridDim.x * 256u)
		cursors[i] = ((unsigned long long)SK_NOCHUNK << 32) | cap;
	for (uint32_t i = blockIdx.x * 256u + threadIdx.x; i < nblk; i += gridDim.x * 256u)
		blk[i] = 0;
}

static __global__ __launch_bounds__(1024) void k_sk_scan(const uint32_t *__restrict__ cnt, uint32_t *__restrict__ off, uint32_t *__restrict__ fillcur,
                                                  int nb, const unsigned long long *__restrict__ kmers, unsigned long long *__restrict__ kpre)
{
	__shared__ unsigned long long s_a[1024], s_b[1024];
	const int t = threadIdx.x, per = (nb + 1023) / 1024;
	const int i0 = t * per, i1 = i0 + per < nb ? i0 + per : nb;
	unsigned long long a = 0, b = 0;
	for (int i = i0; i < i1; i++) {
		a += cnt[i];
		if (kmers) b += kmers[i];
	}
	s_a[t] = a;
	s_b[t] = b;
	__syncthreads();
	for (int d = 1; d < 1024; d <<= 1) {
		const unsigned long long va = t >= d ? s_a[t - d] : 0, vb = t >= d ? s_b[t - d] : 0;
		__syncthreads();
		s_a[t] += va;
		s_b[t] += vb;
		__syncthreads();
	}
	a = t ? s_a[t - 1] : 0;
	b = t ? s_b[t - 1] : 0;
	for (int i = i0; i < i1; i++) {
		off[i] = (uint32_t)a;
		fillcur[i] = 0;
		a += cnt[i];
		if (kmers) {
			kpre[i] = b;
			b += kmers[i];
		}
	}
	if (t == 1023) {
		off[nb] = (uint32_t)s_a[1023];
		if (kmers) kpre[nb] = s_b[1023];
	}
}

static __global__ __launch_bounds__(256) void k_sk_chunk_place(SkPool pool, const uint32_t *__restrict__ off, uint32_t *__restrict__ fillcur,
                                                        uint32_t *__restrict__ list)
{
	const uint32_t used = *pool.next, n = used < pool.chunks ? used : pool.chunks;
	for (uint32_t c = blockIdx.x * 256u + threadIdx.x; c < n; c += gridDim.x * 256u) {
		const uint32_t mt = pool.meta[c];
		if (mt == SK_DEAD)
			continue;
		const uint32_t b = mt & 0xFFFFFFu;
		list[off[b] + atomicAdd(&fillcur[b], 1u)] = c | (((mt >> 24) - 1u) << SK_LIST2_FILL_SHIFT);
	}
}

static __global__ __launch_bounds__(256) void k_sk_chunk_place_few(SkPool pool, const uint32_t *__restrict__ off, uint32_t *__restrict__ fillcur,
                                                            uint32_t *__restrict__ list, int nb)
{
	__shared__ uint32_t s_cnt[1024], s_base[1024];
	constexpr uint32_t STRETCH = 256u * 16u;
	const uint32_t used = *pool.next, n = used < pool.chunks ? used : pool.chunks;
	for (uint32_t c0 = blockIdx.x * STRETCH; c0 < n; c0 += gridDim.x * STRETCH) {
		for (int i = threadIdx.x; i < nb; i += 256)
			s_cnt[i] = 0;
		__syncthreads();
		uint32_t mine[16], bucket[16];
#pragma unroll
		for (int t = 0; t < 16; t++) {
			const uint32_t c = c0 + (uint32_t)t * 256u + threadIdx.x;
			const uint32_t mt = c < n ? pool.meta[c] : SK_DEAD;
			bucket[t] = mt == SK_DEAD ? 0xFFFFFFFFu : (mt & 0xFFFFFFu);
			mine[t] = mt == SK_DEAD ? 0u : atomicAdd(&s_cnt[bucket[t]], 1u);
		}
		__syncthreads();
		for (int i = threadIdx.x; i < nb; i += 256)
			s_base[i] = s_cnt[i] ? atomicAdd(&fillcur[i], s_cnt[i]) : 0u;
		__syncthreads();
#pragma unroll
		for (int t = 0; t < 16; t++)
			if (bucket[t] != 0xFFFFFFFFu)
				list[off[bucket[t]] + s_base[bucket[t]] + mine[t]] = c0 + (uint32_t)t * 256u + threadIdx.x;
		__syncthreads();
	}
}


#ifdef SDT_SK_L2_LOG
__device__ unsigned long long *g_l2_log = nullptr;
__device__ unsigned long long g_l2_log_cap = 0;
#endif

#ifndef SDT_SK_L2S_S1
#define SDT_SK_L2S_S1 4
#endif
#ifndef SDT_SK_L2S_WGS
#define SDT_SK_L2S_WGS 1
#endif
#ifndef SDT_SK_L2S_RPL
#define SDT_SK_L2S_RPL 2
#endif
template <int NW, bool COMPACT = false> struct SkL2Stage {
	static_assert(!COMPACT || NW == 1, "the compact level-2 record is the 1-word keys'");
	static constexpr int S = NW == 1 ? SDT_SK_L2S_S1 : 2;
	static constexpr int GPC = SK_CAP2 / S;
	static constexpr int RPL = NW == 1 ? SDT_SK_L2S_RPL : (NW == 2 ? (SDT_SK_L2S_RPL < 2 ? SDT_SK_L2S_RPL : 2) : 1);
	static constexpr int RWS = COMPACT ? SK_REC2C_WORDS : SkFmt<NW>::REC_WORDS;
	static constexpr int RW2 = COMPACT ? SK_REC2C_WORDS : SkFmt<NW>::REC2_STRIDE;
	static constexpr size_t SMEM = (size_t)SK_NB2 * S * RWS * 8;
};

template <int NW, bool COMPACT> __device__ inline void sk_store_staged(uint64_t *dst, const uint64_t (&rec)[SkL2Stage<NW, COMPACT>::RWS])
{
	if constexpr (COMPACT)
		*reinterpret_cast<ulonglong2 *>(dst) = make_ulonglong2(rec[0], rec[1]);
	else
		sk_store_record2<NW>(dst, rec);
}

template <int NW, bool COMPACT>
__global__ __launch_bounds__(SK_L2S_TPB, SDT_SK_L2S_WGS) void k_sk_scatter_records_staged(SkPool src, const uint32_t *__restrict__ list1,
                                                                         const SkItem *__restrict__ items, SkPool dst,
                                                                         uint32_t *__restrict__ g_cnt, unsigned long long *__restrict__ g_kmers, Stats *stats)
{
	using L2 = SkL2Stage<NW, COMPACT>;
	constexpr int RW = SkFmt<NW>::REC_WORDS, RWS = L2::RWS, RW2 = L2::RW2, S = L2::S, GPC = L2::GPC;
	constexpr int CPT = SK_L2S_TPB / SK_CAP1;
	constexpr int D = L2::RPL;
	extern __shared__ __attribute__((aligned(16))) unsigned long long s_stage[];
	__shared__ uint32_t s_cnt[SK_NB2];
	__shared__ uint32_t s_open[SK_NB2];
	__shared__ uint32_t s_pub_open[SK_NB2], s_pub_new[SK_NB2], s_pub_g[SK_NB2];
	__shared__ unsigned char s_fill[SK_NB2], s_used[SK_NB2];
	__shared__ uint32_t s_kc[SK_NB2], s_cc[SK_NB2];
	__shared__ unsigned long long s_blk;
	const SkItem it = items[blockIdx.x];
	const int tid = threadIdx.x;
	for (int i = tid; i < SK_NB2; i += SK_L2S_TPB) {
		s_cnt[i] = 0;
		s_open[i] = SK_NOCHUNK;
		s_fill[i] = 0;
		s_used[i] = 0;
		s_kc[i] = 0;
		s_cc[i] = 0;
	}
	if (tid == 0)
		s_blk = 0;
	__syncthreads();
	uint32_t failed = 0;
	auto alloc = [&](uint32_t n) -> uint32_t {
		const uint32_t id = sk_alloc_chunks(&s_blk, dst, n, SK_BLK2);
		return id < dst.chunks && id + n <= dst.chunks ? id : SK_NOCHUNK;
	};
	auto slot_of = [&](uint32_t open, uint32_t used, uint32_t first_new, uint32_t t) -> uint64_t * {
		const uint32_t a = (open == SK_NOCHUNK ? (uint32_t)GPC : used) + t / S;
		if (a < (uint32_t)GPC)
			return dst.recs + ((size_t)open * SK_CAP2 + a * S + t % S) * RW2;
		if (first_new == SK_NOCHUNK)
			return nullptr;
		return dst.recs + ((size_t)(first_new + (a - GPC) / GPC) * SK_CAP2 + ((a - GPC) % GPC) * S + t % S) * RW2;
	};
	const uint32_t slot = (uint32_t)tid % SK_CAP1, cfirst = it.c0 + (uint32_t)tid / SK_CAP1;
	uint32_t id_b[D], meta_a[D];
	uint64_t rec_a[D][RW];
	{
		uint32_t id_a[D];
#pragma unroll
		for (int d = 0; d < D; d++) {
			const uint32_t ca = cfirst + (uint32_t)d * CPT, cb = ca + (uint32_t)D * CPT;
			id_a[d] = list1[ca < it.c1 ? ca : it.c0];
			id_b[d] = list1[cb < it.c1 ? cb : it.c0];
		}
#pragma unroll
		for (int d = 0; d < D; d++) {
			const uint32_t ca = cfirst + (uint32_t)d * CPT;
			const uint32_t id = ca < it.c1 ? id_a[d] : 0u;
			meta_a[d] = src.meta[id];
			sk_load_record<RW>(src.recs + ((size_t)id * SK_CAP1 + slot) * RW, rec_a[d]);
		}
	}
	const uint32_t nsweep = (it.c1 - it.c0 + CPT - 1) / CPT;
	for (uint32_t sw = 0; sw < nsweep; sw += (uint32_t)D) {
		uint64_t rec[D][RWS];
		uint32_t b2[D], t[D];
		bool valid[D];
#pragma unroll
		for (int d = 0; d < D; d++) {
			asm volatile("" : "+v"(id_b[d]), "+v"(meta_a[d]));
#pragma unroll
			for (int i = 0; i < RW; i++)
				asm volatile("" : "+v"(rec_a[d][i]));
		}
		uint64_t hdr[D];
		uint32_t fill[D];
#pragma unroll
		for (int d = 0; d < D; d++) {
			const uint32_t ci = cfirst + (sw + (uint32_t)d) * CPT;
			hdr[d] = rec_a[d][0];
			fill[d] = ci < it.c1 ? meta_a[d] >> 24 : 0u;
			if constexpr (COMPACT) {
				sk_pack2(rec_a[d][0], rec_a[d][1], rec_a[d][2], rec[d][0], rec[d][1]);
			} else {
#pragma unroll
				for (int i = 0; i < RW; i++)
					rec[d][i] = rec_a[d][i];
			}
		}
#pragma unroll
		for (int d = 0; d < D; d++) {
			const uint32_t ci = cfirst + (sw + (uint32_t)d) * CPT;
			const uint32_t c1n = ci + (uint32_t)D * CPT, c2n = ci + 2u * (uint32_t)D * CPT;
			const uint32_t id = c1n < it.c1 ? id_b[d] : 0u;
			id_b[d] = list1[c2n < it.c1 ? c2n : it.c0];
			meta_a[d] = src.meta[id];
			sk_load_record<RW>(src.recs + ((size_t)id * SK_CAP1 + slot) * RW, rec_a[d]);
		}
#pragma unroll
		for (int d = 0; d < D; d++) {
			valid[d] = slot < fill[d];
			b2[d] = 0;
			t[d] = 0;
			if (valid[d]) {
				b2[d] = sk_hdr_l2(hdr[d]);
				t[d] = atomicAdd(&s_cnt[b2[d]], 1u);
				atomicAdd(&s_kc[b2[d]], (uint32_t)sk_hdr_n(hdr[d]));
			}
		}
		__syncthreads();
		for (int i = tid; i < SK_NB2; i += SK_L2S_TPB) {
			const uint32_t f = s_fill[i], total = s_cnt[i];
			if (total == f)
				continue;
			const uint32_t G = total / S, left = total - G * S;
			const uint32_t open = s_open[i], used = open == SK_NOCHUNK ? (uint32_t)GPC : s_used[i];
			const uint32_t room = (uint32_t)GPC - used;
			uint32_t first_new = SK_NOCHUNK;
			if (G > room) {
				const uint32_t nnew = (G - room + GPC - 1) / GPC;
				first_new = alloc(nnew);
				if (first_new != SK_NOCHUNK) {
					for (uint32_t j = 0; j < nnew; j++)
						dst.meta[first_new + j] = (it.b1 * SK_NB2 + (uint32_t)i) | ((uint32_t)SK_CAP2 << 24);
					s_cc[i] += nnew;
				}
			}
			s_pub_open[i] = open;
			s_pub_new[i] = first_new;
			s_pub_g[i] = used | (G << 8);
			if (G && f) {
				for (uint32_t j = 0; j < f; j++) {
					uint64_t old[RWS];
#pragma unroll
					for (int w = 0; w < RWS; w++)
						old[w] = s_stage[((size_t)i * S + j) * RWS + w];
					uint64_t *p = slot_of(open, used, first_new, j);
					if (p) sk_store_staged<NW, COMPACT>(p, old);
					else failed++;
				}
			}
			if (G) {
				const uint32_t a_end = used + G;
				if (a_end <= (uint32_t)GPC) {
					s_used[i] = (unsigned char)a_end;
				} else if (first_new != SK_NOCHUNK) {
					s_open[i] = first_new + (a_end - GPC - 1) / GPC;
					s_used[i] = (unsigned char)((a_end - GPC - 1) % GPC + 1);
				} else {
					s_open[i] = SK_NOCHUNK;
					s_used[i] = 0;
				}
			}
			s_fill[i] = (unsigned char)left;
			s_cnt[i] = left;
		}
		__syncthreads();
#pragma unroll
		for (int d = 0; d < D; d++) {
			if (!valid[d])
				continue;
			const uint32_t g = s_pub_g[b2[d]], G = g >> 8, used = g & 0xFFu;
			if (t[d] / S < G) {
				uint64_t *p = slot_of(s_pub_open[b2[d]], used, s_pub_new[b2[d]], t[d]);
				if (p) sk_store_staged<NW, COMPACT>(p, rec[d]);
				else failed++;
			} else {
				const uint32_t at = t[d] - G * S;
#pragma unroll
				for (int i = 0; i < RWS; i++)
					s_stage[((size_t)b2[d] * S + at) * RWS + i] = rec[d][i];
			}
		}
	}
	__syncthreads();
	for (int i = tid; i < SK_NB2; i += SK_L2S_TPB) {
		const uint32_t f = s_fill[i];
		uint32_t open = s_open[i], used = open == SK_NOCHUNK ? (uint32_t)GPC : s_used[i];
		if (f) {
			if (used == (uint32_t)GPC) {
				open = alloc(1);
				used = 0;
				if (open != SK_NOCHUNK)
					s_cc[i]++;
			}
			if (open != SK_NOCHUNK) {
				for (uint32_t j = 0; j < f; j++) {
					uint64_t rec[RWS];
#pragma unroll
					for (int w = 0; w < RWS; w++)
						rec[w] = s_stage[((size_t)i * S + j) * RWS + w];
					sk_store_staged<NW, COMPACT>(dst.recs + ((size_t)open * SK_CAP2 + used * S + j) * RW2, rec);
				}
			} else {
				failed += f;
			}
		}
		if (open != SK_NOCHUNK)
			dst.meta[open] = (it.b1 * SK_NB2 + (uint32_t)i) | ((used * S + f) << 24);
		if (s_kc[i])
			atomicAdd(&g_kmers[it.b1 * SK_NB2 + i], (unsigned long long)s_kc[i]);
		if (s_cc[i])
			atomicAdd(&g_cnt[it.b1 * SK_NB2 + i], s_cc[i]);
	}
	__syncthreads();
	{
		const unsigned long long blk = s_blk;
		const uint32_t next = (uint32_t)blk, end = (uint32_t)(blk >> 32);
		for (uint32_t id = next + (uint32_t)tid; id < end && id < dst.chunks; id += SK_L2S_TPB)
			dst.meta[id] = SK_DEAD;
	}
	if (failed)
		atomicAdd(&stats->probe_fail, (unsigned long long)failed);
}

struct SkGatherPlan {
	uint32_t begin[64];
	uint32_t pre[65];
	uint32_t dst0[64];
	int n, self;
};

template <int RW>
__global__ __launch_bounds__(256) void k_sk_gather(SkPool pool, const uint32_t *__restrict__ list, SkGatherPlan plan,
                                                   uint64_t *__restrict__ send, uint32_t *__restrict__ send_meta,
                                                   uint64_t *__restrict__ recv, uint32_t *__restrict__ recv_meta)
{
	constexpr uint32_t CW = SK_CAP1 * RW;
	const uint32_t total = plan.pre[plan.n], lane = threadIdx.x & 63u;
	for (uint32_t g = blockIdx.x * 4u + (threadIdx.x >> 6); g < total; g += gridDim.x * 4u) {
		int p = 0;
		while (p + 1 < plan.n && plan.pre[p + 1] <= g)
			p++;
		const uint32_t i = g - plan.pre[p];
		const uint32_t chunk = list[plan.begin[p] + i], out = plan.dst0[p] + i;
		const ulonglong2 *s = reinterpret_cast<const ulonglong2 *>(pool.recs + (size_t)chunk * CW);
		ulonglong2 *d = reinterpret_cast<ulonglong2 *>((p == plan.self ? recv : send) + (size_t)out * CW);
		for (uint32_t w = lane; w < CW / 2; w += 64u)
			d[w] = s[w];
		if (lane == 0)
			(p == plan.self ? recv_meta : send_meta)[out] = pool.meta[chunk];
	}
}

static __global__ __launch_bounds__(256) void k_sk_iota(uint32_t *p, uint32_t n)
{
	for (uint32_t i = blockIdx.x * 256u + threadIdx.x; i < n; i += gridDim.x * 256u)
		p[i] = i;
}

template <int NW> __device__ inline uint32_t sk_fold_key(const Key<NW> &k)
{
	uint32_t x = 0;
#pragma unroll
	for (int i = 0; i < NW; i++) {
		x = __builtin_rotateleft32(x, 7) ^ (uint32_t)k.w[i];
		x = __builtin_rotateleft32(x, 9) ^ (uint32_t)(k.w[i] >> 32);
	}
	return x;
}
template <int NW, int SLOTS> __device__ inline uint32_t sk_lds_hash(const Key<NW> &k)
{
	const uint32_t h = sk_fold_key<NW>(k) * 0x9E3779B1u;
	if ((SLOTS & (SLOTS - 1)) == 0)
		return h >> (32 - __builtin_ctz(SLOTS));
	return __umulhi(h, (uint32_t)SLOTS);
}

template <int NW, int SLOTS>
__device__ __forceinline__ int sk_lds_locate(unsigned long long *s_key, uint32_t *s_fill, const Key<NW> &key, uint32_t maxfill, int max_probe = 96)
{
	uint32_t s = sk_lds_hash<NW, SLOTS>(key);
	int found = -2;
	for (int probe = 0; probe < max_probe && found == -2;) {
		uint64_t k0 = __hip_atomic_load(&s_key[s], __ATOMIC_RELAXED, __HIP_MEMORY_SCOPE_WORKGROUP);
		if (k0 == KEY_EMPTY) {
			if (__hip_atomic_load(s_fill, __ATOMIC_RELAXED, __HIP_MEMORY_SCOPE_WORKGROUP) >= maxfill)
				return -1;
			const uint64_t old = atomicCAS(&s_key[s], (unsigned long long)KEY_EMPTY, (unsigned long long)(NW == 1 ? key.w[0] : KEY_LOCKED));
			if (old == KEY_EMPTY) {
				atomicAdd(s_fill, 1u);
				if (NW > 1) {
#pragma unroll
					for (int i = 1; i < NW; i++)
						s_key[i * SLOTS + s] = key.w[i];
					__hip_atomic_store(&s_key[s], key.w[0], __ATOMIC_RELEASE, __HIP_MEMORY_SCOPE_WORKGROUP);
					found = (int)s;
					continue;
				}
				return (int)s;
			}
			k0 = old;
		}
		if (NW > 1 && k0 == KEY_LOCKED)
			continue;
		bool same = k0 == key.w[0];
		if (NW > 1 && same) {
			__builtin_amdgcn_fence(__ATOMIC_ACQUIRE, "workgroup");
#pragma unroll
			for (int i = 1; i < NW; i++)
				same = same && (__hip_atomic_load(&s_key[i * SLOTS + s], __ATOMIC_RELAXED, __HIP_MEMORY_SCOPE_WORKGROUP) == key.w[i]);
		}
		if (same)
			return (int)s;
		s = s + 1 == (uint32_t)SLOTS ? 0u : s + 1;
		probe++;
	}
	return found == -2 ? -1 : found;
}

__device__ inline void sk_lds_update(uint32_t *s_f, int s, uint32_t prev, uint32_t next, uint32_t w)
{
	atomicAdd(&s_f[5 * s + (prev >> 1)], w << ((prev & 1u) << 4));
	atomicAdd(&s_f[5 * s + 4 - (next >> 1)], w << (16u - ((next & 1u) << 4)));
}

__device__ inline uint64_t sk_lds_val(const uint32_t *f)
{
	uint64_t v = 0;
	uint32_t cnt = f[2] & 0xFFFFu;
#pragma unroll
	for (int b = 0; b < 4; b++) {
		const uint32_t l = (f[b >> 1] >> ((b & 1) * 16)) & 0xFFFFu, r = (f[4 - (b >> 1)] >> (16 - (b & 1) * 16)) & 0xFFFFu;
		cnt += l;
		v |= (uint64_t)(l > 63u ? 63u : l) << (6 * b);
		v |= (uint64_t)(r > 63u ? 63u : r) << (24 + 6 * b);
	}
	return v | ((uint64_t)cnt << 48);
}

__device__ inline uint64_t sk_weighted_val(uint32_t w, uint32_t prev, uint32_t next)
{
	const uint64_t c = w > 63u ? 63u : w;
	uint64_t v = (uint64_t)(w & 0xFFFFu) << 48;
	if (prev < 4u) v |= c << (6 * prev);
	if (next < 4u) v |= c << (24 + 6 * next);
	return v;
}

constexpr uint32_t SK_CNT_MAX_SINCE = 65535;

template <int NW, bool TRACK, bool COMPACT>
__global__ __launch_bounds__((SkCntGeo<NW, TRACK>::TPB), (SkCntGeo<NW, TRACK>::WAVES_PER_SIMD)) void k_sk_count(SkPool pool, const uint32_t *__restrict__ list2, const uint4 *__restrict__ items,
                                                         uint32_t item0, uint32_t item1, uint32_t *__restrict__ next_item, int K,
                                                         Table<NW> tbl, Stats *stats)
{
	using G = SkCntGeo<NW, TRACK>;
	constexpr int BW = SkFmt<NW>::BW, RW = SkFmt<NW>::REC_WORDS, SLOTS = G::SLOTS;
	constexpr uint32_t FLUSH_AT = G::FLUSH_AT, MAXFILL = G::MAXFILL;
	constexpr int SK_CNT_TPB = G::TPB;
	constexpr int TR = G::TILE;
	constexpr int CPT = TR / SK_CAP2;
	constexpr int NWAVES = TR / 64;
	constexpr uint32_t REP = G::REP, REP_EMPTY = 0xFFFFFFFFu;
	extern __shared__ unsigned long long sm64[];
	unsigned long long *s_h0 = sm64;
	uint32_t *s_w = (uint32_t *)(s_h0 + TR);
	uint32_t *s_pre = s_w + TR;
	unsigned short *s_map = (unsigned short *)(s_pre + TR + 2);
	unsigned short *s_idx = s_map + TR;
	uint32_t *s_rep = s_pre;
	uint32_t *s_words = (uint32_t *)((char *)s_pre + G::REGION);
	unsigned long long *s_key = (unsigned long long *)(s_words + LDS_LEAD + TR * BW * 2 + TAIL_PAD);
	unsigned long long *s_ord = s_key + NW * SLOTS;
	uint32_t *s_f = (uint32_t *)(s_ord + (TRACK ? SLOTS : 0));
	__shared__ uint32_t s_fillc[2], s_item, s_spilled;
	enum { ST_CLAIMED, ST_FAILED, ST_MERGES, ST_SPILLS, ST_GENS, ST_KMERS, ST_RECS, ST_DRECS, ST_DKMERS, ST_N };
	__shared__ uint32_t s_stat[ST_N];
	__shared__ uint32_t s_ent[3 * (G::TILE / SK_CAP2)];
	__shared__ unsigned long long s_wsum[NWAVES];
	const int tid = threadIdx.x;
	for (int i = tid; i < SLOTS; i += SK_CNT_TPB) {
		s_key[i] = KEY_EMPTY;
		if (TRACK) s_ord[i] = ORD_NONE;
	}
	for (int i = tid; i < 5 * SLOTS; i += SK_CNT_TPB)
		s_f[i] = 0;
	if (tid < LDS_LEAD)
		s_words[tid] = 0;
	if (tid < TAIL_PAD)
		s_words[LDS_LEAD + TR * BW * 2 + tid] = 0;
	if (tid == 0)
		s_fillc[0] = s_fillc[1] = 0;
	if (tid < ST_N)
		s_stat[tid] = 0;
	uint32_t *words = s_words + LDS_LEAD;
#ifdef SDT_SK_TICKS
	unsigned long long cyc[4] = {0, 0, 0, 0}, t0 = wall_clock64(), t1;
#define SK_TICK(i) do { t1 = wall_clock64(); cyc[i] += t1 - t0; t0 = t1; } while (0)
#else
#define SK_TICK(i) do { } while (0)
#endif
	constexpr int PER = (SLOTS + SK_CNT_TPB - 1) / SK_CNT_TPB;
	Key<NW> mk[PER];
	uint64_t madd[PER], mord[TRACK ? PER : 1];
	bool have[PER];
	EntSnap<NW, TRACK> sn[PER];
	uint32_t ko = 0, km = 0;
	uint32_t room_shift = NW == 1 ? 2u : 1u;
	bool stores_pending = false;
	auto flush_finish = [&]() {
		uint32_t claimed = 0, failed = 0, merges = 0;
#pragma unroll
		for (int p = 0; p < PER; p++)
			if (have[p]) {
				merges++;
				if (!table_merge_owned_at<NW, TRACK>(tbl, mk[p], flat_home<NW>(tbl, mk[p]), sn[p], madd[p], 0u, claimed, TRACK ? mord[TRACK ? p : 0] : ORD_NONE))
					failed++;
			}
#pragma unroll
		for (int d = 32; d > 0; d >>= 1) {
			claimed += __shfl_down(claimed, d);
			failed += __shfl_down(failed, d);
			merges += __shfl_down(merges, d);
		}
		if ((tid & 63) == 0) {
			if (claimed) atomicAdd(&s_stat[ST_CLAIMED], claimed);
			if (failed) atomicAdd(&s_stat[ST_FAILED], failed);
			if (merges) atomicAdd(&s_stat[ST_MERGES], merges);
		}
		stores_pending = true;
	};
	for (;;) {
		if (tid == 0) {
			s_item = item0 + atomicAdd(next_item, 1u);
			s_spilled = 0;
		}
		__syncthreads();
		const uint32_t item = (uint32_t)__builtin_amdgcn_readfirstlane((int)s_item);
		__syncthreads();
		if (item >= item1)
			break;
		const uint4 it = items[item];
		const uint32_t ity = (uint32_t)__builtin_amdgcn_readfirstlane((int)it.y);
		const uint32_t c0 = (uint32_t)__builtin_amdgcn_readfirstlane((int)it.x), c1 = ity & 0x7FFFFFFFu;
		const bool whole = (ity >> 31) != 0;
		auto rec_ptr = [&](uint32_t e, uint32_t t) -> const uint64_t * {
			return pool.recs + ((size_t)(e & ((1u << SK_LIST2_FILL_SHIFT) - 1u)) * SK_CAP2 + t % SK_CAP2) * (COMPACT ? SK_REC2C_WORDS : SkFmt<NW>::REC2_STRIDE);
		};
		auto rec_ok = [&](uint32_t e, uint32_t t) -> bool { return e != SK_NOCHUNK && t % SK_CAP2 <= (e >> SK_LIST2_FILL_SHIFT); };
		auto ent_row = [&](uint32_t t) -> uint32_t * { return s_ent + (t % 3u) * CPT; };
		if (tid < CPT) {
			ent_row(0)[tid] = c0 + (uint32_t)tid < c1 ? list2[c0 + tid] : SK_NOCHUNK;
			ent_row(1)[tid] = c0 + CPT + (uint32_t)tid < c1 ? list2[c0 + CPT + tid] : SK_NOCHUNK;
		}
		__syncthreads();
		uint32_t tile_no = 0;
		uint32_t since = 0;
		SK_TICK(0);
		for (uint32_t cb = c0; cb < c1; cb += CPT) {
			uint32_t ot_ = (uint32_t)tid;
			asm volatile("" : "+v"(ot_));
			const int ot = (int)ot_;
			uint32_t n = 0;
			uint64_t h0 = 0;
			uint64_t nx[RW];
			uint32_t ring_e = SK_NOCHUNK, pf = 0;
			const uint32_t e = ot < TR ? ent_row(tile_no)[ot / SK_CAP2] : SK_NOCHUNK;
			const uint32_t e1 = ot < TR ? ent_row(tile_no + 1)[ot / SK_CAP2] : SK_NOCHUNK;
			const bool ok = rec_ok(e, ot);
			ulonglong2 cx = make_ulonglong2(0ULL, 0ULL);
			if constexpr (COMPACT) {
				static_assert(!COMPACT || (NW == 1 && !TRACK), "compact records carry no ordinals");
				cx = *reinterpret_cast<const ulonglong2 *>(ok ? rec_ptr(e, ot) : pool.recs);
			} else {
				sk_load_record<RW>(ok ? rec_ptr(e, ot) : pool.recs, nx);
			}
			const bool ring_ok = ot < CPT && cb + 2 * CPT + (uint32_t)ot < c1;
			ring_e = (list2 + cb)[ring_ok ? 2 * CPT + ot : 0];
			if (!ring_ok)
				ring_e = SK_NOCHUNK;
			if (SDT_SK_PREFETCH)
				pf = *(const uint32_t *)(rec_ok(e1, ot) ? rec_ptr(e1, ot) : pool.recs);
			if constexpr (COMPACT)
				sk_unpack2(cx.x, cx.y, nx[0], nx[1], nx[RW - 1]);
			if (ot < TR) {
				if (ok) {
					h0 = nx[0];
					n = (uint32_t)sk_hdr_n(h0);
#pragma unroll
					for (int i = 0; i < BW; i++) {
						words[ot * BW * 2 + 2 * i] = (uint32_t)(nx[1 + i] >> 32);
						words[ot * BW * 2 + 2 * i + 1] = (uint32_t)nx[1 + i];
					}
				}
				s_h0[ot] = h0;
				s_w[ot] = 1;
			}
			for (uint32_t i = ot; i < REP; i += SK_CNT_TPB)
				s_rep[i] = REP_EMPTY;
			__syncthreads();
			bool distinct = false;
			if (n) {
				distinct = true;
				uint32_t x = (uint32_t)h0 & SK_HDR_KIND_MASK;
#pragma unroll
				for (int i = 0; i < BW; i++) {
					x = __builtin_rotateleft32(x, 5) ^ (uint32_t)nx[1 + i];
					x = __builtin_rotateleft32(x, 11) ^ (uint32_t)(nx[1 + i] >> 32);
				}
				static_assert((REP & (REP - 1)) == 0, "the dedupe slot is the top bits of the hash");
				uint32_t slot = (x * 0x85EBCA77u) >> (32 - __builtin_ctz(REP));
				for (;;) {
					const uint32_t cur = atomicCAS(&s_rep[slot], REP_EMPTY, (uint32_t)ot);
					if (cur == REP_EMPTY)
						break;
					bool same = (((uint32_t)s_h0[cur] ^ (uint32_t)h0) & SK_HDR_KIND_MASK) == 0;
#pragma unroll
					for (int i = 0; i < BW; i++)
						same = same && (((uint64_t)words[cur * BW * 2 + 2 * i] << 32) | words[cur * BW * 2 + 2 * i + 1]) == nx[1 + i];
					if (same) {
						atomicAdd(&s_w[cur], 1u);
						if (TRACK)
							atomicMin(&s_h0[cur], (unsigned long long)h0);
						distinct = false;
						break;
					}
					slot = (slot + 1) & (REP - 1);
				}
			}
			const uint32_t n_mine = distinct ? n : 0u;
			unsigned long long xs = ((unsigned long long)(n ? (n | 0x10000u) : 0u) << 32) | (distinct ? (n | 0x10000u) : 0u);
			const unsigned long long xs_mine = xs;
			if (ot < TR) {
#pragma unroll
				for (int d = 1; d < 64; d <<= 1) {
					const unsigned long long y = __shfl_up(xs, d);
					if ((ot & 63) >= d)
						xs += y;
				}
				if ((ot & 63) == 63)
					s_wsum[ot >> 6] = xs;
			}
			__syncthreads();
			unsigned long long wbase = 0, tot = 0;
#pragma unroll
			for (int wv = 0; wv < NWAVES; wv++) {
				const unsigned long long v = s_wsum[wv];
				if (wv < (ot >> 6)) wbase += v;
				tot += v;
			}
			const uint32_t tlo = (uint32_t)__builtin_amdgcn_readfirstlane((int)(uint32_t)tot), thi = (uint32_t)__builtin_amdgcn_readfirstlane((int)(uint32_t)(tot >> 32));
			const uint32_t total = tlo & 0xFFFFu, ndist = tlo >> 16, tile_kmers = thi & 0xFFFFu;
			bool want_flush = since + tile_kmers > SK_CNT_MAX_SINCE;
			since += tile_kmers;
			if (distinct) {
				const uint32_t ex = (uint32_t)(wbase + xs - xs_mine);
				const uint32_t lo = ex & 0xFFFFu, ci = (ex >> 16) & 0xFFFFu, hi = lo + n_mine;
				s_pre[ci] = lo;
				s_map[ci] = (unsigned short)ot;
				for (uint32_t m16 = (lo + 15u) & ~15u; m16 < hi; m16 += 16u)
					s_idx[m16 >> 4] = (unsigned short)ci;
			}
			if (ot < CPT)
				ent_row(tile_no + 2)[ot] = ring_e;
			asm volatile("" :: "v"(pf));
			if (ot == 0) {
				s_pre[ndist] = total;
				s_stat[ST_KMERS] += tile_kmers;
				s_stat[ST_RECS] += thi >> 16;
				s_stat[ST_DRECS] += ndist;
				s_stat[ST_DKMERS] += total;
			}
			__syncthreads();
			SK_TICK(1);
			const bool last_tile = cb + CPT >= c1;
			tile_no++;
			for (uint32_t qb = 0;;) {
				if (want_flush) {
					SK_TICK(2);
					const bool owned = whole && __builtin_amdgcn_readfirstlane((int)s_spilled) == 0;
					uint32_t claimed = 0, failed = 0, merges = 0;
					if (stores_pending) {
						asm volatile("s_waitcnt vmcnt(0)" ::: "memory");
						__syncthreads();
						stores_pending = false;
					}
					if (owned && (NW > 1 || TRACK) && SDT_SK_SEQ_FLUSH) {
#pragma unroll 1
						for (int i = tid; i < SLOTS; i += SK_CNT_TPB) {
							if (s_key[i] == KEY_EMPTY)
								continue;
							Key<NW> key;
							key.w[0] = s_key[i];
#pragma unroll
							for (int wv = 1; wv < NW; wv++)
								key.w[wv] = s_key[wv * SLOTS + i];
							const uint64_t add = sk_lds_val(&s_f[5 * i]);
							const uint64_t ord = TRACK ? (uint64_t)s_ord[i] : ORD_NONE;
							s_key[i] = KEY_EMPTY;
#pragma unroll
							for (int f = 0; f < 5; f++)
								s_f[5 * i + f] = 0;
							if (TRACK) s_ord[i] = ORD_NONE;
							const uint64_t slot = flat_home<NW>(tbl, key);
							merges++;
							if (!table_merge_owned_at<NW, TRACK>(tbl, key, slot, ent_load<NW, TRACK>(tbl, slot, key, NW == 2 && SDT_SK_CLAIM2_BELOW > 0 && (add >> 48) <= SDT_SK_CLAIM2_BELOW), add, 0u, claimed, ord))
								failed++;
						}
#pragma unroll
						for (int d = 32; d > 0; d >>= 1) {
							claimed += __shfl_down(claimed, d);
							failed += __shfl_down(failed, d);
							merges += __shfl_down(merges, d);
						}
						if ((tid & 63) == 0) {
							if (claimed) atomicAdd(&s_stat[ST_CLAIMED], claimed);
							if (failed) atomicAdd(&s_stat[ST_FAILED], failed);
							if (merges) atomicAdd(&s_stat[ST_MERGES], merges);
						}
						stores_pending = true;
					} else if (owned) {
#pragma unroll
						for (int p = 0; p < PER; p++) {
							const int i = tid + p * SK_CNT_TPB;
							have[p] = i < SLOTS && s_key[i] != KEY_EMPTY;
							if (have[p]) {
								mk[p].w[0] = s_key[i];
#pragma unroll
								for (int wv = 1; wv < NW; wv++)
									mk[p].w[wv] = s_key[wv * SLOTS + i];
								madd[p] = sk_lds_val(&s_f[5 * i]);
								if (TRACK) mord[p] = (uint64_t)s_ord[i];
								s_key[i] = KEY_EMPTY;
#pragma unroll
								for (int f = 0; f < 5; f++)
									s_f[5 * i + f] = 0;
								if (TRACK) s_ord[i] = ORD_NONE;
							}
						}
						__builtin_amdgcn_sched_barrier(0);
						if (NW == 1 && SDT_SK_LOAD16) {
							typedef unsigned int u32x4 __attribute__((ext_vector_type(4)));
							u32x4 raw[PER];
#pragma unroll
							for (int p = 0; p < PER; p++) {
								const Entry<NW> *e = tbl.ent + (have[p] ? flat_home<NW>(tbl, mk[p]) : 0);
								asm volatile("global_load_dwordx4 %0, %1, off sc1" : "=v"(raw[p]) : "v"(e) : "memory");
							}
							asm volatile("s_waitcnt vmcnt(0)" : "+v"(raw[0]) :: "memory");
#pragma unroll
							for (int p = 1; p < PER; p++)
								asm volatile("" : "+v"(raw[p]) :: "memory");
#pragma unroll
							for (int p = 0; p < PER; p++) {
								sn[p].k[0] = ((uint64_t)raw[p].y << 32) | raw[p].x;
								sn[p].v = ((uint64_t)raw[p].w << 32) | raw[p].z;
								sn[p].f = ORD_NONE;
								sn[p].won = false;
							}
						} else {
#pragma unroll
						for (int p = 0; p < PER; p++)
							if (have[p])
								sn[p] = ent_load<NW, TRACK>(tbl, flat_home<NW>(tbl, mk[p]), mk[p], SDT_SK_CLAIM_BELOW > 0 && (madd[p] >> 48) <= SDT_SK_CLAIM_BELOW);
						}
						__builtin_amdgcn_sched_barrier(0);
						flush_finish();
					} else {
						for (int i = tid; i < SLOTS; i += SK_CNT_TPB) {
							const uint64_t k0 = s_key[i];
							if (k0 == KEY_EMPTY)
								continue;
							Key<NW> key;
							key.w[0] = k0;
#pragma unroll
							for (int wv = 1; wv < NW; wv++)
								key.w[wv] = s_key[wv * SLOTS + i];
							merges++;
							const uint64_t add = sk_lds_val(&s_f[5 * i]);
							const uint64_t ord = TRACK ? (uint64_t)s_ord[i] : ORD_NONE;
							if (!table_merge<NW>(tbl, key, add, 0u, claimed, ord))
								failed++;
							s_key[i] = KEY_EMPTY;
#pragma unroll
							for (int f = 0; f < 5; f++)
								s_f[5 * i + f] = 0;
							if (TRACK) s_ord[i] = ORD_NONE;
						}
#pragma unroll
						for (int d = 32; d > 0; d >>= 1) {
							claimed += __shfl_down(claimed, d);
							failed += __shfl_down(failed, d);
							merges += __shfl_down(merges, d);
						}
						if ((tid & 63) == 0) {
							if (claimed) atomicAdd(&s_stat[ST_CLAIMED], claimed);
							if (failed) atomicAdd(&s_stat[ST_FAILED], failed);
#ifdef SDT_SK_SPLIT_MERGE_STAT
							if (merges) atomicAdd(&s_stat[ST_SPILLS], merges);
#else
							if (merges) atomicAdd(&s_stat[ST_MERGES], merges);
#endif
						}
					}
					__syncthreads();
					if (tid == 0) {
						s_fillc[0] = s_fillc[1] = 0;
						if (!(last_tile && qb >= total)) s_stat[ST_GENS]++;
					}
					__syncthreads();
					ko = 0;
					km &= 0x80000000u;
					since = tile_kmers;
					SK_TICK(3);
				}
				if (qb >= total)
					break;
				const uint32_t fill0 = ko + (km & 0x7FFFFFFFu);
				const bool guard = stores_pending;
				const uint32_t room = guard ? (uint32_t)(SLOTS * 3 / 4) : (MAXFILL - fill0) << room_shift;
				const int max_probe = guard ? SLOTS : 96;
				uint32_t *const fillc = &s_fillc[km >> 31];
				const uint32_t maxfill = MAXFILL - ko;
				const uint32_t qe = qb + room < total ? qb + room : total;
				for (uint32_t q = qb + tid; q < qe; q += SK_CNT_TPB) {
					uint32_t ci = s_idx[q >> 4];
					while (s_pre[ci + 1] <= q)
						ci++;
					const int r = s_map[ci];
					const int j = (int)(q - s_pre[ci]);
					const uint64_t hr = s_h0[r];
					const uint32_t wgt = s_w[r];
					const int hp = sk_hdr_prev(hr), nr = sk_hdr_n(hr);
					const int len = hp + nr + K - 1 + sk_hdr_next(hr);
					uint32_t prev, next;
					const Key<NW> key = chop_record<NW>(words, r * BW * 32, len, hp + j, K, prev, next);
					const int s = sk_lds_locate<NW, SLOTS>(s_key, fillc, key, maxfill, max_probe);
					if (s >= 0) {
						sk_lds_update(s_f, s, prev, next, wgt);
						if (TRACK) {
							const uint64_t ord = (sk_hdr_read(hr) << 16) | (uint64_t)(sk_hdr_pos(hr) + (uint32_t)j);
							if (ord < *(volatile unsigned long long *)&s_ord[s])
								atomicMin(&s_ord[s], (unsigned long long)ord);
						}
					} else {
						s_spilled = 1;
						const uint64_t ord = TRACK ? ((sk_hdr_read(hr) << 16) | (uint64_t)(sk_hdr_pos(hr) + (uint32_t)j)) : ORD_NONE;
						uint32_t cl = 0;
						atomicAdd(&s_stat[ST_SPILLS], 1u);
						if (!table_merge<NW>(tbl, key, sk_weighted_val(wgt, prev, next), 0u, cl, ord))
							atomicAdd(&s_stat[ST_FAILED], 1u);
						if (cl)
							atomicAdd(&s_stat[ST_CLAIMED], cl);
					}
				}
				if (guard) {
					asm volatile("s_waitcnt vmcnt(0)" ::: "memory");
					stores_pending = false;
				}
				__syncthreads();
				const uint32_t cur = (uint32_t)__builtin_amdgcn_readfirstlane((int)*fillc);
				const uint32_t fill1 = cur + ko;
				km = ko | (~km & 0x80000000u);
				ko = cur;
				if (NW > 1) {
					if ((fill1 - fill0) * 2u > MAXFILL - fill0)
						room_shift = room_shift ? room_shift - 1u : 0u;
					else if (qe - qb == room && (fill1 - fill0) * 8u < MAXFILL - fill0 && room_shift < 2u)
						room_shift++;
				}
				qb = qe;
				want_flush = (qb >= total && last_tile) || fill1 >= FLUSH_AT;
			}
			SK_TICK(2);
		}
	}
#undef SK_TICK
	__syncthreads();
	if (tid == 0) {
		if (s_stat[ST_CLAIMED]) atomicAdd(&stats->distinct, (unsigned long long)s_stat[ST_CLAIMED]);
		if (s_stat[ST_FAILED]) atomicAdd(&stats->probe_fail, (unsigned long long)s_stat[ST_FAILED]);
		if (s_stat[ST_MERGES]) atomicAdd(&stats->sk_merges, (unsigned long long)s_stat[ST_MERGES]);
		if (s_stat[ST_SPILLS]) atomicAdd(&stats->sk_spills, (unsigned long long)s_stat[ST_SPILLS]);
		if (s_stat[ST_GENS]) atomicAdd(&stats->sk_gens, (unsigned long long)s_stat[ST_GENS]);
		if (s_stat[ST_KMERS]) {
			atomicAdd(&stats->kmers, (unsigned long long)s_stat[ST_KMERS]);
			atomicAdd(&stats->sk_counted, (unsigned long long)s_stat[ST_KMERS]);
		}
		if (s_stat[ST_RECS]) atomicAdd(&stats->sk_records, (unsigned long long)s_stat[ST_RECS]);
		if (s_stat[ST_DRECS]) atomicAdd(&stats->sk_distinct_recs, (unsigned long long)s_stat[ST_DRECS]);
		if (s_stat[ST_DKMERS]) atomicAdd(&stats->sk_distinct_kmers, (unsigned long long)s_stat[ST_DKMERS]);
#ifdef SDT_SK_TICKS
		for (int i = 0; i < 4; i++)
			atomicAdd(&stats->sk_cyc[i], cyc[i]);
#endif
	}
}
```

Baseline: 99.40 billion.

## Pack level-1 super-k-mer records into two words for 1-word keys

Adds a compact level-1 record format for single-word k-mers that folds the L2 bucket, run length and flags into the low bits of the second base word. This drops the record from three 64-bit words to two, cutting write traffic in the scatter kernels and read traffic in the level-2 staged scatter and shard gather. In exchange, the maximum run length is capped by the available base bits, which can produce more and shorter super-k-mers. The non-power-of-two cap check now needs a multiply-high modulo.

```diff
diff --git a/soapdenovo-trans_amd/csrc/sdt_pipeline.hip b/soapdenovo-trans_amd/csrc/sdt_pipeline.hip
--- a/soapdenovo-trans_amd/csrc/sdt_pipeline.hip
+++ b/soapdenovo-trans_amd/csrc/sdt_pipeline.hip
@@ -75,11 +75,11 @@
 		HIPCHK(hipStreamSynchronize(c->stream));
 		sk_free(c);
 	}
-	const bool compact = sk_compact(c);
-	const int rw = sk_rec_words(c->nw), rw2 = sk_rec2_stride(c->nw, compact);
+	const bool compact = sk_compact(c), compact1 = sk_compact_l1(c);
+	const int rw = sk_rec1_words(c), rw2 = sk_rec2_stride(c->nw, compact);
 	const int w = c->K - sk_minimizer_len(c->K) + 1;
 	const bool strips = c->nw == 4 || per_read > (uint64_t)SK_SEQ_MAX_KMERS;
-	const int cap_c = strips ? sk_pow2_floor(sk_max_run(c->K, c->nw, compact)) : sk_max_run(c->K, c->nw, compact);
+	const int cap_c = compact1 ? sk_max_run1(c->K, SK_L2BITS) : (strips ? sk_pow2_floor(sk_max_run(c->K, c->nw, compact)) : sk_max_run(c->K, c->nw, compact));
 	const double rate = 2.0 / (double)(w + 1) + 1.0 / (double)sk_max_run(c->K, c->nw);
 	const double more = compact ? (2.0 / (double)(w + 1) + 1.0 / (double)cap_c) / rate : 1.0;
 	double run = 1.0 / rate * ((c->nw == 4 || per_read > (uint64_t)SK_SEQ_MAX_KMERS) ? 0.8 : 1.0);
@@ -355,7 +355,9 @@
 	sdt_ctx::SkState &k = c->sk;
 	const uint64_t per_read = max_read_len - c->K + 1;
 	const SkGeo geo = sk_geo(c->K, max_read_len);
-	const int m = sk_minimizer_len(c->K), ncap = sk_max_run(c->K, c->nw, sk_compact(c));
+	const bool compact1 = sk_compact_l1(c);
+	const int m = sk_minimizer_len(c->K), ncap = compact1 ? sk_max_run1(c->K, SK_L2BITS) : sk_max_run(c->K, c->nw, sk_compact(c));
+	const int ncap_strips = compact1 ? ncap : sk_pow2_floor(ncap);
 	const uint64_t ntiles = (nr + SK_TILE_READS - 1) / SK_TILE_READS;
 	const unsigned grid = (unsigned)(ntiles < k.wgs ? ntiles : k.wgs);
 	EventPair *ev = next_event(c);
@@ -364,10 +366,10 @@
 	ev->kmers = nr * per_read;
 	ev->stage = SDT_STAGE_SK_SCATTER;
 	HIPCHK(hipEventRecord(ev->a, c->stream));
-#define SK_SCATTER(NW)                                                                                                             \
+#define SK_SCATTER(NW, C1)                                                                                                         \
 	do {                                                                                                                       \
-		HIPCHK(hipFuncSetAttribute((const void *)k_sk_scatter_reads<NW>, hipFuncAttributeMaxDynamicSharedMemorySize, (int)geo.smem)); \
-		hipLaunchKernelGGL(k_sk_scatter_reads<NW>, dim3(grid), dim3(TPB), geo.smem, c->stream, d_words, d_offs, nr, c->K, m, sk_pow2_floor(ncap), \
+		HIPCHK(hipFuncSetAttribute((const void *)k_sk_scatter_reads<NW, C1>, hipFuncAttributeMaxDynamicSharedMemorySize, (int)geo.smem)); \
+		hipLaunchKernelGGL((k_sk_scatter_reads<NW, C1>), dim3(grid), dim3(TPB), geo.smem, c->stream, d_words, d_offs, nr, c->K, m, ncap_strips, \
 		                   geo.mtw, geo.tile_words, geo.hv_words, geo.hv2_words, geo.bits_words, k.p1, k.cursors, k.blk, k.cnt1, sk_tbl<NW>(c, allow_direct), c->d_stats, ob, c->ord_stride); \
 	} while (0)
 	const int w = c->K - m + 1;
@@ -380,11 +382,13 @@
 		a.mtw = (int)(((uint64_t)SK_SEQ_TILE * max_read_len + 16 + 15) / 16) + TAIL_PAD + 1;
 		a.pool = k.p1; a.cursors = k.cursors; a.blk = k.blk; a.cnt = k.cnt1; a.stats = c->d_stats;
 		a.ord_base = ob; a.ord_stride = c->ord_stride; a.max_wgs = k.wgs; a.cu_count = c->cu_count; a.stream = c->stream;
+		a.compact1 = compact1;
 		HIPCHK(seq1 ? sk_seq_launch_nw1(w, a, sk_tbl<1>(c, allow_direct)) : (w <= 33 ? sk_seq_launch_nw2_lo(w, a, sk_tbl<2>(c, allow_direct))
 		            : (w <= 43 ? sk_seq_launch_nw2_mid(w, a, sk_tbl<2>(c, allow_direct)) : sk_seq_launch_nw2_hi(w, a, sk_tbl<2>(c, allow_direct)))));
-	} else if (c->nw == 1) SK_SCATTER(1);
-	else if (c->nw == 2) SK_SCATTER(2);
-	else SK_SCATTER(4);
+	} else if (c->nw == 1 && compact1) SK_SCATTER(1, true);
+	else if (c->nw == 1) SK_SCATTER(1, false);
+	else if (c->nw == 2) SK_SCATTER(2, false);
+	else SK_SCATTER(4, false);
 #undef SK_SCATTER
 	HIPCHK(hipGetLastError());
 	HIPCHK(hipEventRecord(ev->b, c->stream));
diff --git a/soapdenovo-trans_amd/csrc/sdt_pipeline.hpp b/soapdenovo-trans_amd/csrc/sdt_pipeline.hpp
--- a/soapdenovo-trans_amd/csrc/sdt_pipeline.hpp
+++ b/soapdenovo-trans_amd/csrc/sdt_pipeline.hpp
@@ -17,7 +17,8 @@
 	} while (0)
 
 static inline bool sk_compact(const sdt_ctx *c) { return sdt::sk_compact2(c->nw, (c->flags & SDT_FLAG_TRACK_FIRST) != 0); }
-
+static inline bool sk_compact_l1(const sdt_ctx *c) { return sdt::sk_compact1(c->nw, (c->flags & SDT_FLAG_TRACK_FIRST) != 0); }
+static inline int sk_rec1_words(const sdt_ctx *c) { return sdt::sk_rec1_stride(c->nw, sk_compact_l1(c)); }
 struct SkGeo { int mtw, tile_words, hv_words, hv2_words, bits_words; size_t smem; };
 SkGeo sk_geo(int K, uint64_t max_read_len);
 bool sk_applicable(const sdt_ctx *c, uint64_t max_read_len);
diff --git a/soapdenovo-trans_amd/csrc/sdt_scatter_seq_a.hip b/soapdenovo-trans_amd/csrc/sdt_scatter_seq_a.hip
--- a/soapdenovo-trans_amd/csrc/sdt_scatter_seq_a.hip
+++ b/soapdenovo-trans_amd/csrc/sdt_scatter_seq_a.hip
@@ -3,13 +3,13 @@
 hipError_t sk_seq_launch_nw1(int w, const SkSeqLaunch &a, const Table<1> &tbl)
 {
 	switch (w) {
-	case 9: return sk_seq_launch_one<1, 9>(a, tbl);
-	case 11: return sk_seq_launch_one<1, 11>(a, tbl);
-	case 13: return sk_seq_launch_one<1, 13>(a, tbl);
-	case 15: return sk_seq_launch_one<1, 15>(a, tbl);
-	case 17: return sk_seq_launch_one<1, 17>(a, tbl);
-	case 19: return sk_seq_launch_one<1, 19>(a, tbl);
-	case 21: return sk_seq_launch_one<1, 21>(a, tbl);
+	case 9: return a.compact1 ? sk_seq_launch_one<1, 9, true>(a, tbl) : sk_seq_launch_one<1, 9>(a, tbl);
+	case 11: return a.compact1 ? sk_seq_launch_one<1, 11, true>(a, tbl) : sk_seq_launch_one<1, 11>(a, tbl);
+	case 13: return a.compact1 ? sk_seq_launch_one<1, 13, true>(a, tbl) : sk_seq_launch_one<1, 13>(a, tbl);
+	case 15: return a.compact1 ? sk_seq_launch_one<1, 15, true>(a, tbl) : sk_seq_launch_one<1, 15>(a, tbl);
+	case 17: return a.compact1 ? sk_seq_launch_one<1, 17, true>(a, tbl) : sk_seq_launch_one<1, 17>(a, tbl);
+	case 19: return a.compact1 ? sk_seq_launch_one<1, 19, true>(a, tbl) : sk_seq_launch_one<1, 19>(a, tbl);
+	case 21: return a.compact1 ? sk_seq_launch_one<1, 21, true>(a, tbl) : sk_seq_launch_one<1, 21>(a, tbl);
 	default: return hipErrorInvalidValue;
 	}
 }
diff --git a/soapdenovo-trans_amd/csrc/sdt_sharded.hip b/soapdenovo-trans_amd/csrc/sdt_sharded.hip
--- a/soapdenovo-trans_amd/csrc/sdt_sharded.hip
+++ b/soapdenovo-trans_amd/csrc/sdt_sharded.hip
@@ -27,7 +27,7 @@
 		return SDT_OK;
 	HIPCHK(hipStreamSynchronize(c->stream));
 	shard_free(c);
-	const size_t cw = (size_t)SK_CAP1 * sk_rec_words(c->nw) * 8;
+	const size_t cw = (size_t)SK_CAP1 * sk_rec1_words(c) * 8;
 	h.send_chunks = k.p1.chunks;
 	h.recv_chunks = k.p1.chunks + k.p1.chunks / 4;
 	if (sdt_test_env("SDT_SHARD_RECV_CHUNKS"))
@@ -92,7 +92,7 @@
 	auto M = [&](int r, uint32_t b) { return shard_mat(mat.data(), r, b); };
 	const uint32_t *blo = h.ranges;
 	const uint32_t S = shard_subrounds(mat.data(), n, blo, h.recv_chunks);
-	const size_t cw = (size_t)SK_CAP1 * sk_rec_words(c->nw) * 8;
+	const size_t cw = (size_t)SK_CAP1 * sk_rec1_words(c) * 8;
 	for (uint32_t t = 0; t < S; t++) {
 		const int slot = (int)(h.round & 1);
 		ShardRound sr;
@@ -157,7 +157,8 @@
 			HIPCHK(hipStreamWaitEvent(c->stream, h.ev_xdone[slot], 0));
 		if (plan.pre[n]) {
 			const unsigned g = (unsigned)c->cu_count * 8;
-			if (c->nw == 1) hipLaunchKernelGGL(k_sk_gather<SkFmt<1>::REC_WORDS>, dim3(g), dim3(256), 0, c->stream, k.p1, k.list1, plan, h.send[slot], h.send_meta[slot], h.recv[slot], h.recv_meta[slot]);
+			if (sk_rec1_words(c) == SK_REC1C_WORDS) hipLaunchKernelGGL(k_sk_gather<SK_REC1C_WORDS>, dim3(g), dim3(256), 0, c->stream, k.p1, k.list1, plan, h.send[slot], h.send_meta[slot], h.recv[slot], h.recv_meta[slot]);
+			else if (c->nw == 1) hipLaunchKernelGGL(k_sk_gather<SkFmt<1>::REC_WORDS>, dim3(g), dim3(256), 0, c->stream, k.p1, k.list1, plan, h.send[slot], h.send_meta[slot], h.recv[slot], h.recv_meta[slot]);
 			else if (c->nw == 2) hipLaunchKernelGGL(k_sk_gather<SkFmt<2>::REC_WORDS>, dim3(g), dim3(256), 0, c->stream, k.p1, k.list1, plan, h.send[slot], h.send_meta[slot], h.recv[slot], h.recv_meta[slot]);
 			else hipLaunchKernelGGL(k_sk_gather<SkFmt<4>::REC_WORDS>, dim3(g), dim3(256), 0, c->stream, k.p1, k.list1, plan, h.send[slot], h.send_meta[slot], h.recv[slot], h.recv_meta[slot]);
 			HIPCHK(hipGetLastError());
diff --git a/soapdenovo-trans_amd/csrc/sdt_sk_record1.h b/soapdenovo-trans_amd/csrc/sdt_sk_record1.h
--- /dev/null
+++ b/soapdenovo-trans_amd/csrc/sdt_sk_record1.h
@@ -0,0 +1,50 @@
+#pragma once
+#include <stdint.h>
+#include "sdt_sk_record2.h"
+
+namespace sdt {
+
+constexpr int SK_REC1C_WORDS = 2;
+
+#ifndef SDT_SK_COMPACT1
+#define SDT_SK_COMPACT1 1
+#endif
+SDT_SK_HD inline bool sk_compact1(int nw, bool track_first) { return SDT_SK_COMPACT1 && sk_compact2(nw, track_first); }
+
+SDT_SK_HD inline int sk_rec1c_hdr_bits(int l2bits) { return 8 + l2bits; }
+SDT_SK_HD inline uint64_t sk_rec1c_hdr_mask(int l2bits) { return (1ULL << sk_rec1c_hdr_bits(l2bits)) - 1ULL; }
+SDT_SK_HD inline int sk_rec1c_bases(int l2bits) { return 32 + (64 - sk_rec1c_hdr_bits(l2bits)) / 2; }
+
+SDT_SK_HD inline int sk_max_run1(int K, int l2bits)
+{
+	const int n2 = sk_max_run(K, 1, true), n1 = sk_rec1c_bases(l2bits) - K - 1;
+	return n1 < n2 ? n1 : n2;
+}
+
+SDT_SK_HD inline uint64_t sk_rec1c_hdr(uint32_t l2, int n, int has_prev, int has_next, int l2bits)
+{
+	return ((uint64_t)(l2 & ((1u << l2bits) - 1u)) << 8) | ((uint64_t)(n - 1) << 2) | ((uint64_t)has_prev << 1) | (uint64_t)has_next;
+}
+SDT_SK_HD inline void sk_pack1(uint64_t hdr, uint64_t b0, uint64_t b1, int l2bits, uint64_t &w0, uint64_t &w1)
+{
+	const uint64_t m = sk_rec1c_hdr_mask(l2bits);
+	w0 = b0;
+	w1 = (b1 & ~m) | (hdr & m);
+}
+SDT_SK_HD inline void sk_unpack1(uint64_t w0, uint64_t w1, int l2bits, uint64_t &hdr, uint64_t &b0, uint64_t &b1)
+{
+	const uint64_t m = sk_rec1c_hdr_mask(l2bits);
+	hdr = w1 & m;
+	b0 = w0;
+	b1 = w1 & ~m;
+}
+SDT_SK_HD inline uint32_t sk_rec1c_l2(uint64_t w1, int l2bits) { return (uint32_t)(w1 >> 8) & ((1u << l2bits) - 1u); }
+SDT_SK_HD inline int sk_rec1c_n(uint64_t w1) { return (int)((w1 >> 2) & 31u) + 1; }
+
+SDT_SK_HD inline void sk_rec1c_to_rec2c(uint64_t w0, uint64_t w1, int l2bits, uint64_t &v0, uint64_t &v1)
+{
+	v0 = w0;
+	v1 = w1 & ~(sk_rec1c_hdr_mask(l2bits) & ~0xFFULL);
+}
+
+}
diff --git a/soapdenovo-trans_amd/csrc/sdt_sk_scatter_seq.cuh b/soapdenovo-trans_amd/csrc/sdt_sk_scatter_seq.cuh
--- a/soapdenovo-trans_amd/csrc/sdt_sk_scatter_seq.cuh
+++ b/soapdenovo-trans_amd/csrc/sdt_sk_scatter_seq.cuh
@@ -174,7 +174,19 @@
 constexpr int SK_SEQ_MAX_KMERS = 256;
 
 
-template <int NW>
+template <int NW, bool C1> __device__ inline void sk_store_record1(uint64_t *recs, uint32_t chunk, uint32_t pos, const uint64_t (&rec)[SkFmt<NW>::REC_WORDS])
+{
+	if constexpr (C1) {
+		static_assert(NW == 1, "the compact level-1 record is the 1-word keys'");
+		uint64_t w0, w1;
+		sk_pack1(rec[0], rec[1], rec[2], SK_L2BITS, w0, w1);
+		*reinterpret_cast<ulonglong2 *>(recs + ((size_t)chunk * SK_CAP1 + pos) * SK_REC1C_WORDS) = make_ulonglong2(w0, w1);
+	} else {
+		sk_store_record<SkFmt<NW>::REC_WORDS>(recs + ((size_t)chunk * SK_CAP1 + pos) * SkFmt<NW>::REC_WORDS, rec);
+	}
+}
+
+template <int NW, bool C1 = false>
 __device__ inline void sk_emit_run(const uint32_t *words, int rb_r, int len_r, int nk_r, int K, uint64_t read_ord, int j0, int n,
                                    uint32_t fb, unsigned long long *s_cur, unsigned long long *s_blk, const SkPool &pool,
                                    uint32_t *s_cnt, const Table<NW> &tbl, uint32_t &claimed, uint32_t &failed, uint32_t &done,
@@ -187,7 +199,7 @@
 	if (sk_reserve(s_cur, s_blk, l1, l1, SK_CAP1, pool, s_cnt, chunk, pos)) {
 		const int len = hp + n + K - 1 + hn, ps = rb_r + j0 - hp;
 		uint64_t rec[RW];
-		rec[0] = sk_header(read_ord, (uint32_t)j0, l2, n, hp, hn);
+		rec[0] = C1 ? sk_rec1c_hdr(l2, n, hp, hn, SK_L2BITS) : sk_header(read_ord, (uint32_t)j0, l2, n, hp, hn);
 #pragma unroll
 		for (int k = 0; k < BW; k++) {
 			uint64_t wv = 0;
@@ -199,7 +211,7 @@
 			}
 			rec[1 + k] = wv;
 		}
-		sk_store_record<RW>(pool.recs + ((size_t)chunk * SK_CAP1 + pos) * RW, rec);
+		sk_store_record1<NW, C1>(pool.recs, chunk, pos, rec);
 		emitted += (uint32_t)n;
 	} else if (!tbl.ent) {
 		failed += (uint32_t)n;
@@ -215,7 +227,7 @@
 	}
 }
 
-template <int NW, int W>
+template <int NW, int W, bool C1 = false>
 __global__ __launch_bounds__(SK_SEQ_TILE, NW == 1 ? 4 : 2) void k_sk_scatter_reads_seq(const uint32_t *__restrict__ packed, const uint64_t *__restrict__ offs,
                                                                       uint64_t nreads, int K, int m, int ncap, int max_tile_words, SkPool pool,
                                                                       unsigned long long *__restrict__ g_cursors, unsigned long long *__restrict__ g_blk,
@@ -292,7 +304,7 @@
 					if (nrun < SK_SEQ_RUNCAP)
 						runs[nrun] = (fb0 << 6) | (uint32_t)(j - j0 - 1);
 					else
-						sk_emit_run<NW>(words, rb_r, len_r, nk_r, K, read_ord, j0, j - j0, fb0, s_cur, &s_blk, pool, s_cnt, tbl, claimed, failed, done, emitted);
+						sk_emit_run<NW, C1>(words, rb_r, len_r, nk_r, K, read_ord, j0, j - j0, fb0, s_cur, &s_blk, pool, s_cnt, tbl, claimed, failed, done, emitted);
 					nrun++;
 					j0 = j;
 					fb0 = fb;
@@ -329,7 +341,7 @@
 			if (nrun < SK_SEQ_RUNCAP)
 				runs[nrun] = (fb0 << 6) | (uint32_t)(nk_r - j0 - 1);
 			else
-				sk_emit_run<NW>(words, rb_r, len_r, nk_r, K, read_ord, j0, nk_r - j0, fb0, s_cur, &s_blk, pool, s_cnt, tbl, claimed, failed, done, emitted);
+				sk_emit_run<NW, C1>(words, rb_r, len_r, nk_r, K, read_ord, j0, nk_r - j0, fb0, s_cur, &s_blk, pool, s_cnt, tbl, claimed, failed, done, emitted);
 			nrun++;
 		}
 		SK_TICK(1);
@@ -337,7 +349,7 @@
 		for (int k = 0, jr = 0; k < nlist; k++) {
 			const uint32_t e = runs[k];
 			const int nr = (int)(e & 63u) + 1;
-			sk_emit_run<NW>(words, rb_r, len_r, nk_r, K, read_ord, jr, nr, e >> 6, s_cur, &s_blk, pool, s_cnt, tbl, claimed, failed, done, emitted);
+			sk_emit_run<NW, C1>(words, rb_r, len_r, nk_r, K, read_ord, jr, nr, e >> 6, s_cur, &s_blk, pool, s_cnt, tbl, claimed, failed, done, emitted);
 			jr += nr;
 		}
 		__syncthreads();
@@ -383,21 +395,22 @@
 	unsigned max_wgs;
 	int cu_count;
 	hipStream_t stream;
+	bool compact1;
 };
 
-template <int NW, int W> inline hipError_t sk_seq_launch_one(const SkSeqLaunch &a, const Table<NW> &tbl)
+template <int NW, int W, bool C1 = false> inline hipError_t sk_seq_launch_one(const SkSeqLaunch &a, const Table<NW> &tbl)
 {
 	const size_t smem = (size_t)SK_NB1 * 8 + (size_t)(SK_SEQ_TILE + 2) * 4 + (size_t)SK_SEQ_TILE * SK_SEQ_RUNCAP * 4 + (size_t)(LDS_LEAD + a.mtw) * 4;
-	hipError_t e = hipFuncSetAttribute((const void *)k_sk_scatter_reads_seq<NW, W>, hipFuncAttributeMaxDynamicSharedMemorySize, (int)smem);
+	hipError_t e = hipFuncSetAttribute((const void *)k_sk_scatter_reads_seq<NW, W, C1>, hipFuncAttributeMaxDynamicSharedMemorySize, (int)smem);
 	if (e != hipSuccess) return e;
 	int per_cu = 0;
-	e = hipOccupancyMaxActiveBlocksPerMultiprocessor(&per_cu, k_sk_scatter_reads_seq<NW, W>, SK_SEQ_TILE, smem);
+	e = hipOccupancyMaxActiveBlocksPerMultiprocessor(&per_cu, k_sk_scatter_reads_seq<NW, W, C1>, SK_SEQ_TILE, smem);
 	if (e != hipSuccess) return e;
 	uint64_t res = (uint64_t)(per_cu > 0 ? per_cu : 1) * (uint64_t)a.cu_count;
 	if (res > a.max_wgs) res = a.max_wgs;
 	const uint64_t nt = (a.nreads + SK_SEQ_TILE - 1) / SK_SEQ_TILE;
 	const unsigned grid = (unsigned)(nt < res ? nt : res);
-	hipLaunchKernelGGL((k_sk_scatter_reads_seq<NW, W>), dim3(grid), dim3(SK_SEQ_TILE), smem, a.stream, a.words, a.offs, a.nreads, a.K, a.m, a.ncap,
+	hipLaunchKernelGGL((k_sk_scatter_reads_seq<NW, W, C1>), dim3(grid), dim3(SK_SEQ_TILE), smem, a.stream, a.words, a.offs, a.nreads, a.K, a.m, a.ncap,
 	                   a.mtw, a.pool, a.cursors, a.blk, a.cnt, tbl, a.stats, a.ord_base, a.ord_stride);
 	return hipGetLastError();
 }
diff --git a/soapdenovo-trans_amd/csrc/sdt_superkmer.cuh b/soapdenovo-trans_amd/csrc/sdt_superkmer.cuh
--- a/soapdenovo-trans_amd/csrc/sdt_superkmer.cuh
+++ b/soapdenovo-trans_amd/csrc/sdt_superkmer.cuh
@@ -3,6 +3,7 @@
 #include "sdt_minimizer.cuh"
 #include "sdt_table.cuh"
 #include "sdt_sk_record2.h"
+#include "sdt_sk_record1.h"
 
 namespace sdt {
 
@@ -28,6 +29,7 @@
 constexpr int SK_MAX_READ_LEN = (1 << SK_POSBITS) - 1;
 
 __host__ __device__ inline int sk_rec_words(int nw) { return nw == 1 ? 3 : (nw == 2 ? 5 : 7); }
+__host__ __device__ inline int sk_rec1_stride(int nw, bool compact1) { return compact1 ? SK_REC1C_WORDS : sk_rec_words(nw); }
 __host__ __device__ inline int sk_rec2_stride(int nw, bool compact)
 {
 	return compact ? SK_REC2C_WORDS : (nw == 1 ? SkFmt<1>::REC2_STRIDE : (nw == 2 ? SkFmt<2>::REC2_STRIDE : SkFmt<4>::REC2_STRIDE));
diff --git a/soapdenovo-trans_amd/csrc/sdt_superkmer_kernels.cuh b/soapdenovo-trans_amd/csrc/sdt_superkmer_kernels.cuh
--- a/soapdenovo-trans_amd/csrc/sdt_superkmer_kernels.cuh
+++ b/soapdenovo-trans_amd/csrc/sdt_superkmer_kernels.cuh
@@ -59,7 +59,7 @@
 
 #include "sdt_sk_scatter_seq.cuh"
 
-template <int NW>
+template <int NW, bool C1 = false>
 __global__ __launch_bounds__(TPB) void k_sk_scatter_reads(const uint32_t *__restrict__ packed, const uint64_t *__restrict__ offs,
                                                           uint64_t nreads, int K, int m, int ncap, int max_tile_words,
                                                           int tile_smem_words, int hv_words, int hv2_words, int bits_words, SkPool pool,
@@ -86,6 +86,11 @@
 	const int w = K - m + 1;
 	const uint64_t ntiles = (nreads + SK_TILE_READS - 1) / SK_TILE_READS;
 	uint32_t claimed = 0, failed = 0, done = 0, emitted = 0;
+	const bool cap_pow2 = (ncap & (ncap - 1)) == 0;
+	const uint32_t cap_inv = cap_pow2 ? 0u : 0xFFFFFFFFu / (uint32_t)ncap + 1u;
+	auto at_cap = [&](int j) -> bool {
+		return cap_pow2 ? (j & (ncap - 1)) == 0 : (uint32_t)j - __umulhi((uint32_t)j, cap_inv) * (uint32_t)ncap == 0u;
+	};
 #ifdef SDT_SK_TICKS
 	unsigned long long cyc[4] = {0, 0, 0, 0}, t0 = wall_clock64(), t1;
 #define SK_TICK(i) do { t1 = wall_clock64(); cyc[i] += t1 - t0; t0 = t1; } while (0)
@@ -122,7 +127,7 @@
 					const bool kv = lane >= 1 && lane <= valid && j < nk_r;
 					if (kv)
 						s_hv[p] = bh;
-					const bool start = kv && (j == 0 || (j & (ncap - 1)) == 0 || sk_final_bucket(bh) != sk_final_bucket(pbh));
+					const bool start = kv && (j == 0 || at_cap(j) || sk_final_bucket(bh) != sk_final_bucket(pbh));
 					const unsigned long long mask = __ballot(start) >> 1;
 					if (lane == 0 && mask) {
 						const uint32_t q0 = tv.pre[r] + (uint32_t)j0, sh = q0 & 63u;
@@ -160,7 +165,7 @@
 					const int r = tile_find_read(tv.pre, q);
 					const int j = (int)(q - tv.pre[r]);
 					const int p = (int)tv.rb[r] + j;
-					if (j == 0 || (j & (ncap - 1)) == 0) {
+					if (j == 0 || at_cap(j)) {
 						start = true;
 					} else {
 						start = sk_final_bucket(bhs[p]) != sk_final_bucket(bhs[p - 1]);
@@ -228,7 +233,7 @@
 			if (sk_reserve(s_cur, &s_blk, sk_l1_bucket(bh), sk_l1_bucket(bh), SK_CAP1, pool, s_cnt, chunk, pos)) {
 				const int len = hp + n + K - 1 + hn, ps = p0 - hp;
 				uint64_t rec[RW];
-				rec[0] = sk_header(read_ord, (uint32_t)j, sk_l2_bucket(bh), n, hp, hn);
+				rec[0] = C1 ? sk_rec1c_hdr(sk_l2_bucket(bh), n, hp, hn, SK_L2BITS) : sk_header(read_ord, (uint32_t)j, sk_l2_bucket(bh), n, hp, hn);
 #pragma unroll
 				for (int k = 0; k < BW; k++) {
 					uint64_t wv = 0;
@@ -240,7 +245,7 @@
 					}
 					rec[1 + k] = wv;
 				}
-				sk_store_record<RW>(pool.recs + ((size_t)chunk * SK_CAP1 + pos) * RW, rec);
+				sk_store_record1<NW, C1>(pool.recs, chunk, pos, rec);
 				emitted += (uint32_t)n;
 			} else if (!tbl.ent) {
 				failed += (uint32_t)n;
@@ -407,6 +412,8 @@
 	static constexpr int S = NW == 1 ? SDT_SK_L2S_S1 : 2;
 	static constexpr int GPC = SK_CAP2 / S;
 	static constexpr int RPL = NW == 1 ? SDT_SK_L2S_RPL : (NW == 2 ? (SDT_SK_L2S_RPL < 2 ? SDT_SK_L2S_RPL : 2) : 1);
+	static constexpr bool C1 = COMPACT && SDT_SK_COMPACT1;
+	static constexpr int RW1 = C1 ? SK_REC1C_WORDS : SkFmt<NW>::REC_WORDS;
 	static constexpr int RWS = COMPACT ? SK_REC2C_WORDS : SkFmt<NW>::REC_WORDS;
 	static constexpr int RW2 = COMPACT ? SK_REC2C_WORDS : SkFmt<NW>::REC2_STRIDE;
 	static constexpr size_t SMEM = (size_t)SK_NB2 * S * RWS * 8;
@@ -420,13 +427,25 @@
 		sk_store_record2<NW>(dst, rec);
 }
 
+template <int RW1, bool C1> __device__ inline void sk_load_record1(const uint64_t *src, uint64_t (&rec)[RW1])
+{
+	if constexpr (C1) {
+		const ulonglong2 v = *reinterpret_cast<const ulonglong2 *>(src);
+		rec[0] = v.x;
+		rec[1] = v.y;
+	} else {
+		sk_load_record<RW1>(src, rec);
+	}
+}
+
 template <int NW, bool COMPACT>
 __global__ __launch_bounds__(SK_L2S_TPB, SDT_SK_L2S_WGS) void k_sk_scatter_records_staged(SkPool src, const uint32_t *__restrict__ list1,
                                                                          const SkItem *__restrict__ items, SkPool dst,
                                                                          uint32_t *__restrict__ g_cnt, unsigned long long *__restrict__ g_kmers, Stats *stats)
 {
 	using L2 = SkL2Stage<NW, COMPACT>;
-	constexpr int RW = SkFmt<NW>::REC_WORDS, RWS = L2::RWS, RW2 = L2::RW2, S = L2::S, GPC = L2::GPC;
+	constexpr int RW = L2::RW1, RWS = L2::RWS, RW2 = L2::RW2, S = L2::S, GPC = L2::GPC;
+	constexpr bool C1 = L2::C1;
 	constexpr int CPT = SK_L2S_TPB / SK_CAP1;
 	constexpr int D = L2::RPL;
 	extern __shared__ __attribute__((aligned(16))) unsigned long long s_stage[];
@@ -478,7 +497,7 @@
 			const uint32_t ca = cfirst + (uint32_t)d * CPT;
 			const uint32_t id = ca < it.c1 ? id_a[d] : 0u;
 			meta_a[d] = src.meta[id];
-			sk_load_record<RW>(src.recs + ((size_t)id * SK_CAP1 + slot) * RW, rec_a[d]);
+			sk_load_record1<RW, C1>(src.recs + ((size_t)id * SK_CAP1 + slot) * RW, rec_a[d]);
 		}
 	}
 	const uint32_t nsweep = (it.c1 - it.c0 + CPT - 1) / CPT;
@@ -498,9 +517,11 @@
 #pragma unroll
 		for (int d = 0; d < D; d++) {
 			const uint32_t ci = cfirst + (sw + (uint32_t)d) * CPT;
-			hdr[d] = rec_a[d][0];
+			hdr[d] = rec_a[d][C1 ? 1 : 0];
 			fill[d] = ci < it.c1 ? meta_a[d] >> 24 : 0u;
-			if constexpr (COMPACT) {
+			if constexpr (C1) {
+				sk_rec1c_to_rec2c(rec_a[d][0], rec_a[d][1], SK_L2BITS, rec[d][0], rec[d][1]);
+			} else if constexpr (COMPACT) {
 				sk_pack2(rec_a[d][0], rec_a[d][1], rec_a[d][2], rec[d][0], rec[d][1]);
 			} else {
 #pragma unroll
@@ -515,7 +536,7 @@
 			const uint32_t id = c1n < it.c1 ? id_b[d] : 0u;
 			id_b[d] = list1[c2n < it.c1 ? c2n : it.c0];
 			meta_a[d] = src.meta[id];
-			sk_load_record<RW>(src.recs + ((size_t)id * SK_CAP1 + slot) * RW, rec_a[d]);
+			sk_load_record1<RW, C1>(src.recs + ((size_t)id * SK_CAP1 + slot) * RW, rec_a[d]);
 		}
 #pragma unroll
 		for (int d = 0; d < D; d++) {
@@ -523,9 +544,9 @@
 			b2[d] = 0;
 			t[d] = 0;
 			if (valid[d]) {
-				b2[d] = sk_hdr_l2(hdr[d]);
+				b2[d] = C1 ? sk_rec1c_l2(hdr[d], SK_L2BITS) : sk_hdr_l2(hdr[d]);
 				t[d] = atomicAdd(&s_cnt[b2[d]], 1u);
-				atomicAdd(&s_kc[b2[d]], (uint32_t)sk_hdr_n(hdr[d]));
+				atomicAdd(&s_kc[b2[d]], (uint32_t)(C1 ? sk_rec1c_n(hdr[d]) : sk_hdr_n(hdr[d])));
 			}
 		}
 		__syncthreads();
```

After: 102.6 billion, median of 6. 3.2% higher.
